# fatchord/WaveRNN

Hardware: AMD Instinct MI355X
Metric: audio samples/sec (real-time factor @22.05 kHz), MoL WaveRNN batched generate (higher is better)
Workload: dtype f32

## Files before the change

### include/wavernn_amd.h

```cpp
#ifndef WAVERNN_AMD_H
#define WAVERNN_AMD_H

#include <stddef.h>
#include <stdint.h>

#ifdef __cplusplus
extern "C" {
#endif

#define WRNN_ABI_VERSION 9

enum {
    WRNN_OK = 0,
    WRNN_ERR_ARG = -1,
    WRNN_ERR_NO_DEVICE = -2,
    WRNN_ERR_HIP = -3,
    WRNN_ERR_WORKSPACE = -4,
    WRNN_ERR_KERNEL = -5,
    WRNN_ERR_RESIDENCY = -6
};

enum { WRNN_MODE_RAW = 0, WRNN_MODE_MOL = 1 };

enum {
    WRNN_ALGO_AUTO = 0,
    WRNN_ALGO_STREAM = 1,
    WRNN_ALGO_LOOP = 2,
    WRNN_ALGO_DUO = 6,
    WRNN_ALGO_CHAIN = 7,
    WRNN_ALGO_OCTO = 8,
    WRNN_ALGO_SPARSE = 5
};

typedef struct wrnn_weights {
    int32_t rnn_dims;
    int32_t fc_dims;
    int32_t feat_dims;
    int32_t aux_dims;
    int32_t n_classes;
    int32_t mode;
    const float *I_w, *I_b;
    const float *w_ih1, *w_hh1, *b_ih1, *b_hh1;
    const float *w_ih2, *w_hh2, *b_ih2, *b_hh2;
    const float *fc1_w, *fc1_b;
    const float *fc2_w, *fc2_b;
    const float *fc3_w, *fc3_b;
} wrnn_weights;

typedef struct wrnn_pack wrnn_pack;

typedef struct wrnn_geometry {
    int32_t B;
    int32_t T;
    int32_t stride;
    int32_t L;
    int32_t hop;
    int32_t n_frames;
} wrnn_geometry;

typedef struct wrnn_timer wrnn_timer;

typedef struct wrnn_run_info {
    const char *kernel;
    int32_t units_per_wg;
    int32_t clusters;
    int32_t depth;
    int32_t rounds;
    int32_t slab_steps;
    int32_t launches;
} wrnn_run_info;

typedef struct wrnn_options {
    int32_t struct_bytes;
    int32_t algo;
    int32_t depth;
    int32_t clusters;
    int32_t cond_valu;
    int32_t slab_steps;
    int32_t t_begin, t_end;
    int32_t tuning;
    const float *force_x;
    float *logits;
    unsigned long long *phase_clocks;
    wrnn_timer *timer;
    wrnn_run_info *info;
    void (*progress)(int32_t steps_done, int32_t T, int32_t n_segments, void *user);
    void *progress_user;
    int32_t mel_stage;
    int32_t mel_rows;
    int32_t mel_scale;
    const float *mel_taps;
    const int32_t *seg_moff;
} wrnn_options;

const char *wrnn_last_error(void);
int wrnn_abi_version(void);

int wrnn_device_cus(int device);

int wrnn_pack_create(const wrnn_weights *w, int device, wrnn_pack **out);
void wrnn_pack_destroy(wrnn_pack *p);
size_t wrnn_pack_weight_bytes(const wrnn_pack *p);
int wrnn_pack_sparse_blocks(const wrnn_pack *p);
int wrnn_pack_sparse_fc_blocks(const wrnn_pack *p);

size_t wrnn_workspace_bytes(const wrnn_pack *p, const wrnn_geometry *g, const wrnn_options *opt);

int wrnn_generate(const wrnn_pack *p, const wrnn_geometry *g, const float *mels_up, const float *aux,
                  const float *noise, float *out, void *workspace, size_t workspace_bytes, const wrnn_options *opt,
                  void *stream);

int wrnn_generate_segments(const wrnn_pack *p, int32_t n_segments, int32_t T, const int32_t *seg_pos,
                           const int32_t *seg_lim, int32_t L, int32_t hop, int32_t n_frames,
                           const float *mels_up, const float *aux, const float *noise, float *out,
                           void *workspace, size_t workspace_bytes, const wrnn_options *opt, void *stream);
size_t wrnn_workspace_bytes_segments(const wrnn_pack *p, int32_t n_segments, int32_t T, int32_t n_frames,
                                     const wrnn_options *opt);

int wrnn_plan_segments(const wrnn_pack *p, int32_t n_segments, int32_t T, const wrnn_options *opt, wrnn_run_info *out);

int wrnn_status(void *workspace, void *stream);

int wrnn_debug_read_exchange(const wrnn_pack *p, void *workspace, int32_t n_segments, int32_t T, int32_t n_frames,
                             const wrnn_options *opt, int cluster, int slot, int layer, int ring, float *host_out);

int wrnn_timer_create(int device, wrnn_timer **out);
void wrnn_timer_destroy(wrnn_timer *t);
float wrnn_timer_ms(wrnn_timer *t);
int wrnn_timer_launches(const wrnn_timer *t);

typedef struct wrnn_pre_weights {
    int32_t feat_dims;
    int32_t compute_dims;
    int32_t res_out_dims;
    int32_t res_blocks;
    int32_t pad;
    int32_t upsample_factors[3];
    const float *conv_in_w;
    const float *bn_in;
    const float *res_w;
    const float *res_bn;
    const float *conv_out_w;
    const float *conv_out_b;
    const float *up_w;
} wrnn_pre_weights;
typedef struct wrnn_pre wrnn_pre;

int wrnn_pre_create(const wrnn_pre_weights *w, int device, wrnn_pre **out);
void wrnn_pre_destroy(wrnn_pre *p);
int wrnn_pre_hop(const wrnn_pre *p);
size_t wrnn_pre_workspace_bytes(const wrnn_pre *p, int32_t n_frames);
int wrnn_pre_upsample(const wrnn_pre *p, const float *mel, int32_t n_frames, float *mels_up, float *aux,
                      void *workspace, size_t workspace_bytes, void *stream);
int wrnn_pre_upsample_rows(const wrnn_pre *p, const float *mel, int32_t n_frames, float *mel_rows, float *aux,
                           void *workspace, size_t workspace_bytes, void *stream);
const char *wrnn_pre_last_error(void);

int wrnn_post_unfold(const float *segments, int32_t T, int32_t n_utt, const int32_t *first, const int32_t *folds,
                     const int64_t *out_off, const double *lut, int32_t n_classes, const double *fade_in,
                     const double *fade_out, int32_t overlap, const double *tail, int32_t tail_len, int32_t batched,
                     double *out, void *stream);
const char *wrnn_post_last_error(void);

typedef struct wrnn_taco_weights {
    uint32_t struct_bytes;
    int32_t n_mels, prenet1, prenet2, decoder_dims, encoder_width, lstm_dims, attn_filters, attn_kernel;
    const float *prenet_fc1_w, *prenet_fc1_b, *prenet_fc2_w, *prenet_fc2_b;
    const float *attn_rnn_w_ih, *attn_rnn_w_hh, *attn_rnn_b_ih, *attn_rnn_b_hh;
    const float *attn_W_w, *attn_W_b, *attn_conv_w, *attn_L_w, *attn_L_b, *attn_v_w;
    const float *rnn_input_w, *rnn_input_b;
    const float *rnn1_w_ih, *rnn1_w_hh, *rnn1_b_ih, *rnn1_b_hh;
    const float *rnn2_w_ih, *rnn2_w_hh, *rnn2_b_ih, *rnn2_b_hh;
    const float *mel_proj_w;
} wrnn_taco_weights;

typedef struct wrnn_taco_call {
    uint32_t struct_bytes;
    int32_t n;
    int32_t r, max_r;
    int32_t max_steps;
    float stop_threshold;
    const float *seq;
    const float *seq_proj;
    float *mel_out;
    float *scores_out;
    int32_t *steps_done;
    void *workspace;
    size_t workspace_bytes;
    void *stream;
    int32_t variant;
} wrnn_taco_call;

size_t wrnn_taco_workspace_bytes(void);
int wrnn_taco_decode(int device, const wrnn_taco_weights *w, const wrnn_taco_call *c);
int wrnn_taco_status(const void *workspace, unsigned *out4, void *stream);
const char *wrnn_taco_last_error(void);

typedef struct wrnn_bigru_call {
    uint32_t struct_bytes;
    int32_t T, hidden;
    const float *gi_fwd, *gi_rev;
    const float *w_hh_fwd, *w_hh_rev;
    const float *b_hh_fwd, *b_hh_rev;
    float *out;
    void *stream;
} wrnn_bigru_call;
int wrnn_bigru(int device, const wrnn_bigru_call *c);

int wrnn_selftest(int device, int which);
float wrnn_selftest_metric(void);

#ifdef __cplusplus
}
#endif
#endif
```

### wavernn_amd/_lib.py

```python
import ctypes
import os
import subprocess

_HERE = os.path.dirname(os.path.abspath(__file__))
CSRC = os.path.join(_HERE, 'csrc')
SO_PATH = os.path.join(CSRC, 'libwavernn_amd.so')

WRNN_OK = 0
ERR_RESIDENCY = -6
MODE_RAW, MODE_MOL = 0, 1
ABI_VERSION = 9
ALGO_AUTO, ALGO_STREAM, ALGO_LOOP, ALGO_SPARSE, ALGO_DUO, ALGO_CHAIN, ALGO_OCTO = 0, 1, 2, 5, 6, 7, 8
ALGOS = {'auto': ALGO_AUTO, 'stream': ALGO_STREAM, 'loop': ALGO_LOOP, 'sparse': ALGO_SPARSE, 'duo': ALGO_DUO, 'chain': ALGO_CHAIN, 'octo': ALGO_OCTO}

EXPORTS = ['wrnn_last_error', 'wrnn_abi_version', 'wrnn_device_cus', 'wrnn_pack_create', 'wrnn_pack_destroy',
           'wrnn_pack_weight_bytes', 'wrnn_pack_sparse_blocks', 'wrnn_pack_sparse_fc_blocks', 'wrnn_workspace_bytes', 'wrnn_workspace_bytes_segments', 'wrnn_generate',
           'wrnn_generate_segments', 'wrnn_plan_segments', 'wrnn_status', 'wrnn_timer_create', 'wrnn_timer_destroy', 'wrnn_timer_ms',
           'wrnn_timer_launches', 'wrnn_debug_read_exchange', 'wrnn_selftest', 'wrnn_selftest_metric', 'wrnn_pre_create',
           'wrnn_pre_destroy', 'wrnn_pre_hop', 'wrnn_pre_workspace_bytes', 'wrnn_pre_upsample', 'wrnn_pre_upsample_rows', 'wrnn_pre_last_error',
           'wrnn_post_unfold', 'wrnn_post_last_error', 'wrnn_taco_workspace_bytes', 'wrnn_taco_decode', 'wrnn_taco_status',
           'wrnn_taco_last_error', 'wrnn_bigru']


class Weights(ctypes.Structure):
    _fields_ = [(n, ctypes.c_int32) for n in ('rnn_dims', 'fc_dims', 'feat_dims', 'aux_dims', 'n_classes', 'mode')] + \
               [(n, ctypes.c_void_p) for n in ('I_w', 'I_b', 'w_ih1', 'w_hh1', 'b_ih1', 'b_hh1', 'w_ih2', 'w_hh2',
                                               'b_ih2', 'b_hh2', 'fc1_w', 'fc1_b', 'fc2_w', 'fc2_b', 'fc3_w', 'fc3_b')]


class PreWeights(ctypes.Structure):
    _fields_ = [(n, ctypes.c_int32) for n in ('feat_dims', 'compute_dims', 'res_out_dims', 'res_blocks', 'pad')] + \
               [('upsample_factors', ctypes.c_int32 * 3)] + \
               [(n, ctypes.c_void_p) for n in ('conv_in_w', 'bn_in', 'res_w', 'res_bn', 'conv_out_w', 'conv_out_b', 'up_w')]


TACO_WEIGHT_FIELDS = ('prenet_fc1_w', 'prenet_fc1_b', 'prenet_fc2_w', 'prenet_fc2_b', 'attn_rnn_w_ih', 'attn_rnn_w_hh', 'attn_rnn_b_ih',
                      'attn_rnn_b_hh', 'attn_W_w', 'attn_W_b', 'attn_conv_w', 'attn_L_w', 'attn_L_b', 'attn_v_w', 'rnn_input_w', 'rnn_input_b',
                      'rnn1_w_ih', 'rnn1_w_hh', 'rnn1_b_ih', 'rnn1_b_hh', 'rnn2_w_ih', 'rnn2_w_hh', 'rnn2_b_ih', 'rnn2_b_hh', 'mel_proj_w')


class TacoWeights(ctypes.Structure):
    _fields_ = [('struct_bytes', ctypes.c_uint32)] + \
               [(n, ctypes.c_int32) for n in ('n_mels', 'prenet1', 'prenet2', 'decoder_dims', 'encoder_width', 'lstm_dims', 'attn_filters',
                                              'attn_kernel')] + \
               [(n, ctypes.c_void_p) for n in TACO_WEIGHT_FIELDS]


class TacoCall(ctypes.Structure):
    _fields_ = [('struct_bytes', ctypes.c_uint32), ('n', ctypes.c_int32), ('r', ctypes.c_int32), ('max_r', ctypes.c_int32),
                ('max_steps', ctypes.c_int32), ('stop_threshold', ctypes.c_float), ('seq', ctypes.c_void_p), ('seq_proj', ctypes.c_void_p),
                ('mel_out', ctypes.c_void_p), ('scores_out', ctypes.c_void_p), ('steps_done', ctypes.c_void_p),
                ('workspace', ctypes.c_void_p), ('workspace_bytes', ctypes.c_size_t), ('stream', ctypes.c_void_p), ('variant', ctypes.c_int32)]


class BigruCall(ctypes.Structure):
    _fields_ = [('struct_bytes', ctypes.c_uint32), ('T', ctypes.c_int32), ('hidden', ctypes.c_int32)] + \
               [(n, ctypes.c_void_p) for n in ('gi_fwd', 'gi_rev', 'w_hh_fwd', 'w_hh_rev', 'b_hh_fwd', 'b_hh_rev', 'out', 'stream')]


class Geometry(ctypes.Structure):
    _fields_ = [(n, ctypes.c_int32) for n in ('B', 'T', 'stride', 'L', 'hop', 'n_frames')]


class RunInfo(ctypes.Structure):
    _fields_ = [('kernel', ctypes.c_char_p)] + \
               [(n, ctypes.c_int32) for n in ('units_per_wg', 'clusters', 'depth', 'rounds', 'slab_steps', 'launches')]


class Options(ctypes.Structure):
    _fields_ = [(n, ctypes.c_int32) for n in ('struct_bytes', 'algo', 'depth', 'clusters', 'cond_valu', 'slab_steps', 't_begin',
                                              't_end', 'tuning')] + \
               [('force_x', ctypes.c_void_p), ('logits', ctypes.c_void_p), ('phase_clocks', ctypes.c_void_p), ('timer', ctypes.c_void_p),
                ('info', ctypes.POINTER(RunInfo)), ('progress', ctypes.c_void_p), ('progress_user', ctypes.c_void_p),
                ('mel_stage', ctypes.c_int32), ('mel_rows', ctypes.c_int32), ('mel_scale', ctypes.c_int32),
                ('mel_taps', ctypes.c_void_p), ('seg_moff', ctypes.c_void_p)]

    def __init__(self, **kw):
        super().__init__(**kw)
        self.struct_bytes = ctypes.sizeof(Options)


PROGRESS_FN = ctypes.CFUNCTYPE(None, ctypes.c_int32, ctypes.c_int32, ctypes.c_int32, ctypes.c_void_p)


class WrnnError(RuntimeError):
    pass


class ResidencyError(WrnnError):
    """WRNN_ERR_RESIDENCY on the FIRST slice of a step-sliced `auto` run: the persistent grid is not co-resident right now.  The
    callers that slice (WaveRNN.generate, generate_corpus) catch it and redo the call unsliced on the stream kernel."""


def build(verbose=False):
    cmd = [os.path.join(CSRC, 'build.sh')]
    res = subprocess.run(cmd, stdout=subprocess.PIPE, stderr=subprocess.STDOUT, text=True)
    if verbose or res.returncode != 0:
        print(res.stdout)
    if res.returncode != 0:
        raise WrnnError('building libwavernn_amd.so failed')
    global _lib
    _lib = None
    return SO_PATH


_lib = None


def lib():
    global _lib
    if _lib is not None:
        return _lib
    if not os.path.exists(SO_PATH):
        raise WrnnError(f'{SO_PATH} not found: run `python -c "import __graft_entry__ as g; g.build()"` '
                        f'(or wavernn_amd/csrc/build.sh).  There is no CPU fallback.')
    import torch
    L = ctypes.CDLL(SO_PATH)
    L.wrnn_last_error.restype = ctypes.c_char_p
    L.wrnn_abi_version.restype = ctypes.c_int
    L.wrnn_device_cus.argtypes = [ctypes.c_int]
    L.wrnn_pack_create.argtypes = [ctypes.POINTER(Weights), ctypes.c_int, ctypes.POINTER(ctypes.c_void_p)]
    L.wrnn_pack_destroy.argtypes = [ctypes.c_void_p]
    L.wrnn_pack_destroy.restype = None
    L.wrnn_pack_weight_bytes.argtypes = [ctypes.c_void_p]
    L.wrnn_pack_weight_bytes.restype = ctypes.c_size_t
    L.wrnn_pack_sparse_blocks.argtypes = [ctypes.c_void_p]
    L.wrnn_pack_sparse_fc_blocks.argtypes = [ctypes.c_void_p]
    L.wrnn_workspace_bytes.argtypes = [ctypes.c_void_p, ctypes.POINTER(Geometry), ctypes.POINTER(Options)]
    L.wrnn_workspace_bytes.restype = ctypes.c_size_t
    L.wrnn_generate.argtypes = [ctypes.c_void_p, ctypes.POINTER(Geometry), ctypes.c_void_p, ctypes.c_void_p,
                                ctypes.c_void_p, ctypes.c_void_p, ctypes.c_void_p, ctypes.c_size_t, ctypes.POINTER(Options),
                                ctypes.c_void_p]
    L.wrnn_workspace_bytes_segments.argtypes = [ctypes.c_void_p, ctypes.c_int32, ctypes.c_int32, ctypes.c_int32,
                                                ctypes.POINTER(Options)]
    L.wrnn_workspace_bytes_segments.restype = ctypes.c_size_t
    L.wrnn_generate_segments.argtypes = [ctypes.c_void_p, ctypes.c_int32, ctypes.c_int32, ctypes.c_void_p, ctypes.c_void_p,
                                         ctypes.c_int32, ctypes.c_int32, ctypes.c_int32, ctypes.c_void_p, ctypes.c_void_p,
                                         ctypes.c_void_p, ctypes.c_void_p, ctypes.c_void_p, ctypes.c_size_t,
                                         ctypes.POINTER(Options), ctypes.c_void_p]
    L.wrnn_plan_segments.argtypes = [ctypes.c_void_p, ctypes.c_int32, ctypes.c_int32, ctypes.POINTER(Options), ctypes.POINTER(RunInfo)]
    L.wrnn_timer_create.argtypes = [ctypes.c_int, ctypes.POINTER(ctypes.c_void_p)]
    L.wrnn_timer_destroy.argtypes = [ctypes.c_void_p]
    L.wrnn_timer_destroy.restype = None
    L.wrnn_timer_ms.argtypes = [ctypes.c_void_p]
    L.wrnn_timer_ms.restype = ctypes.c_float
    L.wrnn_timer_launches.argtypes = [ctypes.c_void_p]
    L.wrnn_debug_read_exchange.argtypes = [ctypes.c_void_p, ctypes.c_void_p, ctypes.c_int32, ctypes.c_int32, ctypes.c_int32,
                                           ctypes.POINTER(Options), ctypes.c_int, ctypes.c_int, ctypes.c_int, ctypes.c_int,
                                           ctypes.c_void_p]
    L.wrnn_pre_create.argtypes = [ctypes.POINTER(PreWeights), ctypes.c_int, ctypes.POINTER(ctypes.c_void_p)]
    L.wrnn_pre_destroy.argtypes = [ctypes.c_void_p]
    L.wrnn_pre_destroy.restype = None
    L.wrnn_pre_hop.argtypes = [ctypes.c_void_p]
    L.wrnn_pre_workspace_bytes.argtypes = [ctypes.c_void_p, ctypes.c_int32]
    L.wrnn_pre_workspace_bytes.restype = ctypes.c_size_t
    L.wrnn_pre_upsample.argtypes = [ctypes.c_void_p, ctypes.c_void_p, ctypes.c_int32, ctypes.c_void_p, ctypes.c_void_p,
                                    ctypes.c_void_p, ctypes.c_size_t, ctypes.c_void_p]
    L.wrnn_pre_upsample_rows.argtypes = L.wrnn_pre_upsample.argtypes
    L.wrnn_pre_last_error.restype = ctypes.c_char_p
    L.wrnn_post_unfold.argtypes = [ctypes.c_void_p, ctypes.c_int32, ctypes.c_int32, ctypes.c_void_p, ctypes.c_void_p, ctypes.c_void_p,
                                   ctypes.c_void_p, ctypes.c_int32, ctypes.c_void_p, ctypes.c_void_p, ctypes.c_int32,
                                   ctypes.c_void_p, ctypes.c_int32, ctypes.c_int32, ctypes.c_void_p, ctypes.c_void_p]
    L.wrnn_post_last_error.restype = ctypes.c_char_p
    L.wrnn_taco_workspace_bytes.restype = ctypes.c_size_t
    L.wrnn_taco_decode.argtypes = [ctypes.c_int, ctypes.POINTER(TacoWeights), ctypes.POINTER(TacoCall)]
    L.wrnn_taco_status.argtypes = [ctypes.c_void_p, ctypes.POINTER(ctypes.c_uint32 * 4), ctypes.c_void_p]
    L.wrnn_taco_last_error.restype = ctypes.c_char_p
    L.wrnn_bigru.argtypes = [ctypes.c_int, ctypes.POINTER(BigruCall)]
    L.wrnn_status.argtypes = [ctypes.c_void_p, ctypes.c_void_p]
    L.wrnn_selftest.argtypes = [ctypes.c_int, ctypes.c_int]
    L.wrnn_selftest_metric.restype = ctypes.c_float
    _lib = L
    return L


def check(rc, what):
    if rc != WRNN_OK:
        raise WrnnError(f'{what} failed (rc={rc}): {lib().wrnn_last_error().decode()}')
```

### wavernn_amd/csrc/wrnn_abi.hip

```cpp
#include <hip/hip_runtime.h>
#include <stdarg.h>
#include <stdio.h>
#include <stdlib.h>
#include <string.h>
#include <math.h>
#include <string>
#include <vector>

#include "../../include/wavernn_amd.h"
#include "wrnn_device.h"

namespace wrnn {
hipError_t launch_cond(const CondArgs &a, int n_cus, bool valu, hipStream_t stream);
hipError_t launch_cond_frames(const CondArgs &a, hipStream_t stream);
hipError_t launch_cond_frames_slab(const CondArgs &a, hipStream_t stream);
hipError_t launch_cond_frag(const CondArgs &a, int n_cus, hipStream_t stream);
hipError_t launch_noise_mol(const float *in, float *out, long n, int B, int n_cus, hipStream_t stream);
hipError_t launch_stream(const LoopArgs &args, int mode, hipStream_t stream);
hipError_t launch_loop(const LoopArgs &args, int ncl, int mode, hipStream_t stream);
int loop_max_depth(int mode);
int loop_clusters(int n_cus);
size_t loop_state_floats(int G);
hipError_t launch_generic(const GenArgs &args, int mode, hipStream_t stream);
bool generic_dims_ok(int H, int F, int M, int A, int C, int mode);
hipError_t launch_duo(const LoopArgs &args, int ncl, int mode, hipStream_t stream);
int duo_clusters(int n_cus);
int duo_max_depth();
size_t duo_xbuf_bytes(int G);
size_t duo_xbuf_bytes_max();
hipError_t launch_sparse(const LoopArgs &args, int nbp, int mode, hipStream_t stream);
int sparse_clusters(int n_cus);
size_t sparse_state_floats();
size_t sparse_xbuf_bytes();
hipError_t launch_put_floats(float *dst, const float *src, int n, hipStream_t stream);
hipError_t launch_chain(const LoopArgs &args, int mode, hipStream_t stream);
hipError_t launch_octo(const LoopArgs &args, int ncl, int mode, hipStream_t stream);
int octo_clusters(int n_cus);
int octo_max_depth();
int chain_clusters(int n_cus);
int chain_max_depth();
size_t chain_state_floats(int G);
size_t chain_xbuf_bytes(int G);
int selftest_mfma(char *msg, size_t n);
int selftest_allgather(int n_cus, char *msg, size_t n, float *us_per_round);
int selftest_tanh(char *msg, size_t n);
int selftest_xor(char *msg, size_t n);
}

using namespace wrnn;

static thread_local char g_err[512] = "";
static void set_err(const char *fmt, ...)
{
    va_list ap;
    va_start(ap, fmt);
    vsnprintf(g_err, sizeof g_err, fmt, ap);
    va_end(ap);
}
#define HIPCHK(expr)                                                                          \
    do {                                                                                      \
        hipError_t e_ = (expr);                                                               \
        if (e_ != hipSuccess) {                                                               \
            set_err("%s failed: %s (%s:%d)", #expr, hipGetErrorString(e_), __FILE__, __LINE__); \
            return WRNN_ERR_HIP;                                                              \
        }                                                                                     \
    } while (0)

struct wrnn_pack {
    int device, n_cus, C, mode;
    size_t weight_bytes;
    char *dev;
    size_t dev_bytes;
    const float *I_w0, *I_b, *I_cT;
    const float *w_ih1, *w_hh1, *b_ih1, *b_hh1, *w_ih2, *w_hh2, *b_ih2, *b_hh2;
    const float *fc1_w, *fc1_b, *fc2_w, *fc2_b, *fc3_w, *fc3_b;
    const float *w_ih1T, *w_hh1T, *w_ih2T, *w_hh2T, *fc1T, *fc2T, *fc3T, *c2_wT, *c3_wT, *c4_wT;
    const float *fc3f;
    const float *u1;
    bool generic;
    int gH, gF, gM, gA;
    const float *g_I_T, *g_fc1T, *g_fc2T, *g_w_ih2T;
    int sp_nbp;
    int sp_max_blocks;
    const float *sp_vals;
    const int *sp_cols;
    int sp_fc_max_blocks;
    const float *sp_fc_vals;
    const int *sp_fc_cols;
};

extern "C" const char *wrnn_last_error(void) { return g_err; }
extern "C" int wrnn_abi_version(void) { return WRNN_ABI_VERSION; }

extern "C" int wrnn_device_cus(int device)
{
    int n = 0;
    if (hipGetDeviceCount(&n) != hipSuccess || n <= 0 || device >= n) {
        set_err("no HIP device %d (count %d)", device, n);
        return WRNN_ERR_NO_DEVICE;
    }
    hipDeviceProp_t prop;
    if (hipGetDeviceProperties(&prop, device) != hipSuccess) return WRNN_ERR_NO_DEVICE;
    return prop.multiProcessorCount;
}

namespace {
struct Builder {
    std::vector<float> host;
    size_t add(const float *src, size_t n)
    {
        size_t off = (host.size() + 63) / 64 * 64;
        host.resize(off + n);
        if (src) memcpy(host.data() + off, src, n * sizeof(float));
        return off;
    }
    size_t add_T(const float *src, int rows, int ld, int col0, int ncols)
    {
        size_t off = add(nullptr, (size_t)ncols * rows);
        float *d = host.data() + off;
        for (int r = 0; r < rows; ++r)
            for (int k = 0; k < ncols; ++k) d[(size_t)k * rows + r] = src[(size_t)r * ld + col0 + k];
        return off;
    }
};
}

extern "C" int wrnn_pack_create(const wrnn_weights *w, int device, wrnn_pack **out)
{
    if (!w || !out) { set_err("NULL argument"); return WRNN_ERR_ARG; }
    const bool shipped = w->rnn_dims == H && w->fc_dims == H && w->feat_dims == MEL && w->aux_dims == AUX;
    const int C = w->n_classes;
    if (w->mode == WRNN_MODE_MOL) {
        if (C != 30) { set_err("MOL needs n_classes == 30"); return WRNN_ERR_ARG; }
    } else if (w->mode == WRNN_MODE_RAW) {
        if (shipped && (C < 2 || C > H)) { set_err("RAW needs 2 <= n_classes <= 512 with the shipped dims"); return WRNN_ERR_ARG; }
    } else { set_err("unknown mode %d", w->mode); return WRNN_ERR_ARG; }
    if (!shipped && !generic_dims_ok(w->rnn_dims, w->fc_dims, w->feat_dims, w->aux_dims, C, w->mode)) {
        set_err("unsupported dims rnn=%d fc=%d feat=%d aux=%d classes=%d: the generic kernel takes rnn, fc, classes <= 2048, feat + aux <= 1024 "
                "(MOL: 30 classes)", w->rnn_dims, w->fc_dims, w->feat_dims, w->aux_dims, C);
        return WRNN_ERR_ARG;
    }
    const float *const *ptrs = &w->I_w;
    for (int i = 0; i < 16; ++i)
        if (!ptrs[i]) { set_err("NULL weight pointer #%d", i); return WRNN_ERR_ARG; }
    const int cus = wrnn_device_cus(device);
    if (cus < 0) return cus;
    DeviceGuard dg(device);
    HIPCHK(dg.err);

    if (!shipped) {
        const int gH = w->rnn_dims, gF = w->fc_dims, gM = w->feat_dims, gA = w->aux_dims;
        Builder b;
        const size_t oI = b.add_T(w->I_w, gH, 1 + gM + gA, 0, 1 + gM + gA), oIb = b.add(w->I_b, gH);
        const size_t o1i = b.add_T(w->w_ih1, 3 * gH, gH, 0, gH), o1h = b.add_T(w->w_hh1, 3 * gH, gH, 0, gH);
        const size_t o1bi = b.add(w->b_ih1, 3 * gH), o1bh = b.add(w->b_hh1, 3 * gH);
        const size_t o2i = b.add_T(w->w_ih2, 3 * gH, gH + gA, 0, gH + gA), o2h = b.add_T(w->w_hh2, 3 * gH, gH, 0, gH);
        const size_t o2bi = b.add(w->b_ih2, 3 * gH), o2bh = b.add(w->b_hh2, 3 * gH);
        const size_t of1 = b.add_T(w->fc1_w, gF, gH + gA, 0, gH + gA), of1b = b.add(w->fc1_b, gF);
        const size_t of2 = b.add_T(w->fc2_w, gF, gF + gA, 0, gF + gA), of2b = b.add(w->fc2_b, gF);
        const size_t of3 = b.add_T(w->fc3_w, C, gF, 0, gF), of3b = b.add(w->fc3_b, C);
        b.add(nullptr, 64);
        wrnn_pack *p = new wrnn_pack();
        memset(p, 0, sizeof *p);
        p->device = device; p->n_cus = cus; p->C = C; p->mode = w->mode; p->generic = true;
        p->gH = gH; p->gF = gF; p->gM = gM; p->gA = gA;
        p->dev_bytes = b.host.size() * sizeof(float);
        p->weight_bytes = sizeof(float) * ((size_t)gH * (1 + gM + gA) + gH + 2 * ((size_t)3 * gH * gH) + (size_t)3 * gH * (gH + gA) + (size_t)3 * gH * gH +
                                           4 * 3 * gH + (size_t)gF * (gH + gA) + (size_t)gF * (gF + gA) + 2 * gF + (size_t)C * gF + C);
        hipError_t e = hipMalloc((void **)&p->dev, p->dev_bytes);
        if (e != hipSuccess) { set_err("hipMalloc(%zu) failed: %s", p->dev_bytes, hipGetErrorString(e)); delete p; return WRNN_ERR_HIP; }
        e = hipMemcpy(p->dev, b.host.data(), p->dev_bytes, hipMemcpyHostToDevice);
        if (e != hipSuccess) { set_err("hipMemcpy failed: %s", hipGetErrorString(e)); (void)hipFree(p->dev); delete p; return WRNN_ERR_HIP; }
        const float *base = (const float *)p->dev;
        p->g_I_T = base + oI; p->I_b = base + oIb;
        p->w_ih1T = base + o1i; p->w_hh1T = base + o1h; p->b_ih1 = base + o1bi; p->b_hh1 = base + o1bh;
        p->g_w_ih2T = base + o2i; p->w_hh2T = base + o2h; p->b_ih2 = base + o2bi; p->b_hh2 = base + o2bh;
        p->g_fc1T = base + of1; p->fc1_b = base + of1b; p->g_fc2T = base + of2; p->fc2_b = base + of2b;
        p->fc3T = base + of3; p->fc3_b = base + of3b;
        p->sp_max_blocks = gH;
        *out = p;
        return WRNN_OK;
    }

    const int KI = 1 + MEL + AUX, K2 = H + AUX;
    Builder b;
    std::vector<float> col0(H);
    for (int r = 0; r < H; ++r) col0[r] = w->I_w[(size_t)r * KI];
    const size_t o_I_w0 = b.add(col0.data(), H), o_I_b = b.add(w->I_b, H);
    const size_t o_I_cT = b.add_T(w->I_w, H, KI, 1, KCOND);
    const size_t o_w_ih1 = b.add(w->w_ih1, (size_t)3 * H * H), o_w_hh1 = b.add(w->w_hh1, (size_t)3 * H * H);
    const size_t o_b_ih1 = b.add(w->b_ih1, 3 * H), o_b_hh1 = b.add(w->b_hh1, 3 * H);
    const size_t o_w_ih2 = b.add(w->w_ih2, (size_t)3 * H * K2), o_w_hh2 = b.add(w->w_hh2, (size_t)3 * H * H);
    const size_t o_b_ih2 = b.add(w->b_ih2, 3 * H), o_b_hh2 = b.add(w->b_hh2, 3 * H);
    const size_t o_fc1_w = b.add(w->fc1_w, (size_t)H * K2), o_fc1_b = b.add(w->fc1_b, H);
    const size_t o_fc2_w = b.add(w->fc2_w, (size_t)H * K2), o_fc2_b = b.add(w->fc2_b, H);
    const size_t o_fc3_w = b.add(w->fc3_w, (size_t)C * H), o_fc3_b = b.add(w->fc3_b, C);
    const size_t o_w_ih1T = b.add_T(w->w_ih1, 3 * H, H, 0, H), o_w_hh1T = b.add_T(w->w_hh1, 3 * H, H, 0, H);
    const size_t o_w_ih2T = b.add_T(w->w_ih2, 3 * H, K2, 0, H), o_w_hh2T = b.add_T(w->w_hh2, 3 * H, H, 0, H);
    const size_t o_fc1T = b.add_T(w->fc1_w, H, K2, 0, H), o_fc2T = b.add_T(w->fc2_w, H, K2, 0, H);
    const size_t o_fc3T = b.add_T(w->fc3_w, C, H, 0, H);
    const size_t o_c2_wT = b.add_T(w->w_ih2, 3 * H, K2, H, AUX);
    const size_t o_c3_wT = b.add_T(w->fc1_w, H, K2, H, AUX), o_c4_wT = b.add_T(w->fc2_w, H, K2, H, AUX);
    size_t o_fc3f = 0;
    if (w->mode == WRNN_MODE_MOL) {
        o_fc3f = b.add(nullptr, (size_t)2 * SEG * H);
        for (int q = 0; q < 2 * SEG * H / 4; ++q) {
            const int l6 = q & 63, r = (q >> 6) & 7, wv = (q >> 9) & 3, tile = q >> 11;
            const int row = 16 * tile + (l6 & 15), kq = l6 >> 4;
            for (int e = 0; e < 4; ++e)
                b.host[o_fc3f + (size_t)q * 4 + e] = row < C ? w->fc3_w[(size_t)row * H + 128 * wv + 16 * r + 4 * kq + e] : 0.f;
        }
    }
    size_t o_u1 = 0;
    {
        o_u1 = b.add(nullptr, (size_t)3 * H);
        for (int r = 0; r < 3 * H; ++r) {
            double acc = 0.0;
            for (int k = 0; k < H; ++k) acc += (double)w->w_ih1[(size_t)r * H + k] * (double)col0[k];
            b.host[o_u1 + r] = (float)acc;
        }
    }
    int sp_nbp = 0, sp_max = 0, sp_fc_max = 0;
    bool sp_fc_ok = false;
    size_t o_spv = 0, o_spc = 0, o_sfv = 0, o_sfc = 0;
    {
        const float *mats[4] = {w->w_ih1, w->w_hh1, w->w_ih2, w->w_hh2};
        const int lds_[4] = {H, H, K2, H};
        std::vector<std::vector<int>> cols((size_t)4 * 32 * 3);
        for (int m = 0; m < 4; ++m)
            for (int wg = 0; wg < 32; ++wg)
                for (int g = 0; g < 3; ++g) {
                    std::vector<int> &cv = cols[((size_t)m * 32 + wg) * 3 + g];
                    const float *base = mats[m] + ((size_t)g * H + 16 * wg) * lds_[m];
                    for (int c = 0; c < H; ++c) {
                        bool nz = false;
                        for (int r = 0; r < 16 && !nz; ++r) nz = base[(size_t)r * lds_[m] + c] != 0.0f;
                        if (nz) cv.push_back(c);
                    }
                    if ((int)cv.size() > sp_max) sp_max = (int)cv.size();
                }
        const float *fmats[2] = {w->fc1_w, w->fc2_w};
        std::vector<std::vector<int>> fcols((size_t)2 * 32);
        for (int m = 0; m < 2; ++m)
            for (int wg = 0; wg < 32; ++wg) {
                std::vector<int> &cv = fcols[(size_t)m * 32 + wg];
                const float *base = fmats[m] + (size_t)(16 * wg) * K2;
                for (int c = 0; c < H; ++c) {
                    bool nz = false;
                    for (int r = 0; r < 16 && !nz; ++r) nz = base[(size_t)r * K2 + c] != 0.0f;
                    if (nz) cv.push_back(c);
                }
                if ((int)cv.size() > sp_fc_max) sp_fc_max = (int)cv.size();
            }
        if (sp_max <= 64 && (w->mode == WRNN_MODE_MOL || C == H)) {
            sp_nbp = sp_max <= 48 ? 48 : 64;
            if (sp_fc_max <= 64) {
                if (sp_fc_max > 48) sp_nbp = 64;
                o_sfv = b.add(nullptr, (size_t)2 * 32 * sp_nbp * 16);
                o_sfc = b.add(nullptr, (size_t)2 * 32 * sp_nbp);
                for (size_t q = 0; q < (size_t)2 * 32 * sp_nbp * 16; ++q) b.host[o_sfv + q] = 0.f;
                int *fi_ = reinterpret_cast<int *>(b.host.data() + o_sfc);
                for (size_t q = 0; q < (size_t)2 * 32 * sp_nbp; ++q) fi_[q] = 0;
                for (int m = 0; m < 2; ++m)
                    for (int wg = 0; wg < 32; ++wg) {
                        const size_t br = (size_t)m * 32 + wg;
                        const std::vector<int> &cv = fcols[br];
                        const float *base = fmats[m] + (size_t)(16 * wg) * K2;
                        for (size_t k = 0; k < cv.size(); ++k) {
                            reinterpret_cast<int *>(b.host.data() + o_sfc)[br * sp_nbp + k] = cv[k];
                            for (int r = 0; r < 16; ++r) b.host[o_sfv + (br * sp_nbp + k) * 16 + r] = base[(size_t)r * K2 + cv[k]];
                        }
                    }
                sp_fc_ok = true;
            }
            o_spv = b.add(nullptr, (size_t)4 * 32 * 3 * sp_nbp * 16);
            o_spc = b.add(nullptr, (size_t)4 * 32 * 3 * sp_nbp);
            for (size_t q = 0; q < (size_t)4 * 32 * 3 * sp_nbp * 16; ++q) b.host[o_spv + q] = 0.f;
            int *ci = reinterpret_cast<int *>(b.host.data() + o_spc);
            for (size_t q = 0; q < (size_t)4 * 32 * 3 * sp_nbp; ++q) ci[q] = 0;
            for (int m = 0; m < 4; ++m)
                for (int wg = 0; wg < 32; ++wg)
                    for (int g = 0; g < 3; ++g) {
                        const size_t br = ((size_t)m * 32 + wg) * 3 + g;
                        const std::vector<int> &cv = cols[br];
                        const float *base = mats[m] + ((size_t)g * H + 16 * wg) * lds_[m];
                        for (size_t k = 0; k < cv.size(); ++k) {
                            ci[br * sp_nbp + k] = cv[k];
                            for (int r = 0; r < 16; ++r) b.host[o_spv + (br * sp_nbp + k) * 16 + r] = base[(size_t)r * lds_[m] + cv[k]];
                        }
                    }
        }
    }
    b.add(nullptr, 64);

    wrnn_pack *p = new wrnn_pack();
    p->device = device; p->n_cus = cus; p->C = C; p->mode = w->mode;
    p->dev_bytes = b.host.size() * sizeof(float);
    p->weight_bytes = sizeof(float) * ((size_t)H * KI + H + 2 * ((size_t)3 * H * H) + (size_t)3 * H * K2 + (size_t)3 * H * H +
                                       4 * 3 * H + 2 * ((size_t)H * K2 + H) + (size_t)C * H + C);
    hipError_t e = hipMalloc((void **)&p->dev, p->dev_bytes);
    if (e != hipSuccess) { set_err("hipMalloc(%zu) failed: %s", p->dev_bytes, hipGetErrorString(e)); delete p; return WRNN_ERR_HIP; }
    e = hipMemcpy(p->dev, b.host.data(), p->dev_bytes, hipMemcpyHostToDevice);
    if (e != hipSuccess) { set_err("hipMemcpy failed: %s", hipGetErrorString(e)); (void)hipFree(p->dev); delete p; return WRNN_ERR_HIP; }
    const float *base = (const float *)p->dev;
    p->I_w0 = base + o_I_w0; p->I_b = base + o_I_b; p->I_cT = base + o_I_cT;
    p->w_ih1 = base + o_w_ih1; p->w_hh1 = base + o_w_hh1; p->b_ih1 = base + o_b_ih1; p->b_hh1 = base + o_b_hh1;
    p->w_ih2 = base + o_w_ih2; p->w_hh2 = base + o_w_hh2; p->b_ih2 = base + o_b_ih2; p->b_hh2 = base + o_b_hh2;
    p->fc1_w = base + o_fc1_w; p->fc1_b = base + o_fc1_b; p->fc2_w = base + o_fc2_w; p->fc2_b = base + o_fc2_b;
    p->fc3_w = base + o_fc3_w; p->fc3_b = base + o_fc3_b;
    p->w_ih1T = base + o_w_ih1T; p->w_hh1T = base + o_w_hh1T; p->w_ih2T = base + o_w_ih2T; p->w_hh2T = base + o_w_hh2T;
    p->fc1T = base + o_fc1T; p->fc2T = base + o_fc2T; p->fc3T = base + o_fc3T;
    p->c2_wT = base + o_c2_wT; p->c3_wT = base + o_c3_wT; p->c4_wT = base + o_c4_wT;
    p->fc3f = w->mode == WRNN_MODE_MOL ? base + o_fc3f : nullptr;
    p->u1 = base + o_u1;
    p->sp_nbp = sp_nbp; p->sp_max_blocks = sp_max;
    p->sp_vals = sp_nbp ? base + o_spv : nullptr;
    p->sp_cols = sp_nbp ? reinterpret_cast<const int *>(base + o_spc) : nullptr;
    p->sp_fc_max_blocks = sp_fc_max;
    p->sp_fc_vals = sp_fc_ok ? base + o_sfv : nullptr;
    p->sp_fc_cols = sp_fc_ok ? reinterpret_cast<const int *>(base + o_sfc) : nullptr;
    *out = p;
    return WRNN_OK;
}

extern "C" void wrnn_pack_destroy(wrnn_pack *p)
{
    if (!p) return;
    (void)hipFree(p->dev);
    delete p;
}

extern "C" size_t wrnn_pack_weight_bytes(const wrnn_pack *p) { return p ? p->weight_bytes : 0; }

extern "C" int wrnn_pack_sparse_blocks(const wrnn_pack *p) { return p ? (p->sp_nbp ? p->sp_max_blocks : -p->sp_max_blocks) : 0; }
extern "C" int wrnn_pack_sparse_fc_blocks(const wrnn_pack *p) { return p ? (p->sp_fc_vals ? p->sp_fc_max_blocks : -p->sp_fc_max_blocks) : 0; }

struct wrnn_timer {
    int device;
    std::vector<hipEvent_t> ev;
    int used;
};

extern "C" int wrnn_timer_create(int device, wrnn_timer **out)
{
    if (!out) { set_err("NULL argument"); return WRNN_ERR_ARG; }
    const int cus = wrnn_device_cus(device);
    if (cus < 0) return cus;
    wrnn_timer *t = new wrnn_timer();
    t->device = device;
    t->used = 0;
    *out = t;
    return WRNN_OK;
}

extern "C" void wrnn_timer_destroy(wrnn_timer *t)
{
    if (!t) return;
    for (hipEvent_t e : t->ev) (void)hipEventDestroy(e);
    delete t;
}

extern "C" int wrnn_timer_launches(const wrnn_timer *t) { return t ? t->used / 2 : 0; }

extern "C" float wrnn_timer_ms(wrnn_timer *t)
{
    if (!t || t->used < 2) return -1.f;
    float total = 0.f;
    for (int i = 0; i + 1 < t->used; i += 2) {
        if (hipEventSynchronize(t->ev[i + 1]) != hipSuccess) return -1.f;
        float ms = 0.f;
        if (hipEventElapsedTime(&ms, t->ev[i], t->ev[i + 1]) != hipSuccess) return -1.f;
        total += ms;
    }
    return total;
}

namespace {
int timer_mark(wrnn_timer *t, hipStream_t stream)
{
    if (!t) return WRNN_OK;
    if (t->used == (int)t->ev.size()) {
        hipEvent_t e;
        HIPCHK(hipEventCreate(&e));
        t->ev.push_back(e);
    }
    HIPCHK(hipEventRecord(t->ev[t->used], stream));
    t->used += 1;
    return WRNN_OK;
}

struct ProgressCtx {
    void (*fn)(int32_t, int32_t, int32_t, void *);
    void *user;
    int32_t done, T, n;
};
void progress_trampoline(void *p)
{
    ProgressCtx *c = static_cast<ProgressCtx *>(p);
    c->fn(c->done, c->T, c->n, c->user);
    delete c;
}
int enqueue_progress(const wrnn_options *o, int done, int T, int n, hipStream_t stream)
{
    if (!o->progress) return WRNN_OK;
    ProgressCtx *c = new ProgressCtx{o->progress, o->progress_user, done, T, n};
    hipError_t e = hipLaunchHostFunc(stream, progress_trampoline, c);
    if (e != hipSuccess) {
        delete c;
        set_err("hipLaunchHostFunc failed: %s", hipGetErrorString(e));
        return WRNN_ERR_HIP;
    }
    return WRNN_OK;
}

enum Kind { K_STREAM, K_LOOP, K_SPARSE, K_DUO, K_GENERIC, K_CHAIN };
constexpr int DUO_TAB_FPS = 8;
constexpr bool DUO_AUTO = true;
constexpr int CHAIN_AUTO_GROUPS = 8;
constexpr bool OCTO_AUTO = false;
constexpr int DUO_MIN_DEPTH = 1;

struct Plan {
    Kind kind;
    int ncl, G, rounds, per_round, slab, ngr_max;
    int tab_fps;
    int t0, t1;
    bool octo;
};

struct WsLayout {
    size_t status, xcc, segs, melc, c2f, c3f, c4f;
    size_t cI, npre;
    size_t xbuf, state, cIf;
    size_t total;
};
size_t al(size_t x) { return (x + 255) / 256 * 256; }

const wrnn_options *norm_options(const wrnn_options *opt, wrnn_options *tmp)
{
    memset(tmp, 0, sizeof *tmp);
    if (opt) {
        size_t n = opt->struct_bytes > 0 ? (size_t)opt->struct_bytes : sizeof *tmp;
        if (n > sizeof *tmp) n = sizeof *tmp;
        memcpy(tmp, opt, n);
    }
    tmp->struct_bytes = (int32_t)sizeof *tmp;
    return tmp;
}

int make_plan(const wrnn_pack *p, int B, int T, const wrnn_options *o, Plan *pl)
{
    const bool shape_ok = (p->mode == WRNN_MODE_MOL) || (p->C == H);
    pl->t0 = o->t_begin; pl->t1 = o->t_end;
    if (pl->t0 == 0 && pl->t1 == 0) pl->t1 = T;
    if (pl->t0 < 0 || pl->t1 > T || pl->t0 >= pl->t1) { set_err("bad step range [%d, %d) of T=%d", pl->t0, pl->t1, T); return WRNN_ERR_ARG; }
    const int algo = o->algo;
    pl->octo = false;
    if (algo != WRNN_ALGO_AUTO && algo != WRNN_ALGO_STREAM && algo != WRNN_ALGO_LOOP && algo != WRNN_ALGO_SPARSE && algo != WRNN_ALGO_DUO && algo != WRNN_ALGO_CHAIN &&
        algo != WRNN_ALGO_OCTO) {
        set_err("unknown algo %d", algo);
        return WRNN_ERR_ARG;
    }
    const int groups = (B + SEG - 1) / SEG;
    pl->kind = K_STREAM; pl->ncl = 0; pl->G = 0; pl->rounds = 1; pl->per_round = B; pl->slab = T; pl->ngr_max = groups;
    if (p->generic) {
        if (algo != WRNN_ALGO_AUTO && algo != WRNN_ALGO_STREAM) {
            set_err("this pack has non-shipped dims (rnn %d, fc %d, feat %d, aux %d): only the generic kernel (algo auto / stream) runs it", p->gH, p->gF, p->gM, p->gA);
            return WRNN_ERR_ARG;
        }
        if (pl->t0 != 0 || pl->t1 != T) { set_err("a partial step range needs a persistent loop kernel"); return WRNN_ERR_ARG; }
        pl->kind = K_GENERIC;
        return WRNN_OK;
    }
    const int ccl = chain_clusters(p->n_cus);
    const bool chain_hw = shape_ok && ccl >= 1;
    if (algo == WRNN_ALGO_CHAIN && !chain_hw) {
        set_err("wrnn_chain_kernel needs MOL or RAW with 512 classes, and >= 256 CUs (C = %d, device: %d CUs)", p->C, p->n_cus);
        return !shape_ok ? WRNN_ERR_ARG : WRNN_ERR_RESIDENCY;
    }
    const bool sparse_auto = p->sp_nbp && p->mode == WRNN_MODE_MOL;
    if (algo == WRNN_ALGO_CHAIN || (algo == WRNN_ALGO_AUTO && chain_hw && groups <= CHAIN_AUTO_GROUPS && !sparse_auto)) {
        const int gmax = chain_max_depth();
        int g = o->depth;
        if (g < 1 || g > gmax) {
            const int rounds = (groups + ccl * gmax - 1) / (ccl * gmax);
            g = (groups + ccl * rounds - 1) / (ccl * rounds);
            if (g < 1) g = 1;
            if (g > gmax) g = gmax;
        }
        pl->kind = K_CHAIN; pl->ncl = ccl; pl->G = g;
        pl->rounds = (groups + ccl * g - 1) / (ccl * g);
        pl->per_round = (B + pl->rounds - 1) / pl->rounds;
        pl->ngr_max = (pl->per_round + SEG - 1) / SEG;
        if (pl->ngr_max > ccl * g) { pl->rounds += 1; pl->per_round = (B + pl->rounds - 1) / pl->rounds; pl->ngr_max = (pl->per_round + SEG - 1) / SEG; }
        int slab = o->slab_steps;
        if (slab < 1) {
            slab = p->mode == WRNN_MODE_MOL ? (int)((32u << 20) / ((size_t)pl->per_round * 11 * sizeof(float) * pl->rounds)) : 4096;
            if (slab < 16) slab = 16;
            if (slab > 4096) slab = 4096;
        }
        if (slab > T) slab = T;
        pl->slab = slab;
        pl->tab_fps = DUO_TAB_FPS;
    }
    const int scl = sparse_clusters(p->n_cus);
    if (algo == WRNN_ALGO_SPARSE && (!p->sp_nbp || scl < 1)) {
        set_err("block-sparse kernel needs MOL or RAW with 512 classes, >= 256 CUs and GRU matrices with <= 64 surviving 16x1 blocks per block row "
                "(this pack: mode %s, %d classes, up to %d blocks; device: %d CUs)", p->mode == WRNN_MODE_MOL ? "MOL" : "RAW", p->C, p->sp_max_blocks, p->n_cus);
        return (!p->sp_nbp) ? WRNN_ERR_ARG : WRNN_ERR_RESIDENCY;
    }
    if (pl->kind == K_CHAIN) {
    } else if (algo == WRNN_ALGO_SPARSE || (algo == WRNN_ALGO_AUTO && sparse_auto && scl >= 1)) {
        pl->kind = K_SPARSE; pl->ncl = scl; pl->G = 1;
        pl->rounds = (groups + scl - 1) / scl;
        pl->per_round = (B + pl->rounds - 1) / pl->rounds;
        pl->ngr_max = (pl->per_round + SEG - 1) / SEG;
        if (pl->ngr_max > scl) { pl->rounds += 1; pl->per_round = (B + pl->rounds - 1) / pl->rounds; pl->ngr_max = (pl->per_round + SEG - 1) / SEG; }
        int slab = o->slab_steps;
        if (slab < 1) {
            slab = p->mode == WRNN_MODE_MOL ? (int)((32u << 20) / ((size_t)pl->per_round * 11 * sizeof(float) * pl->rounds)) : 4096;
            if (slab < 16) slab = 16;
            if (slab > 4096) slab = 4096;
        }
        if (slab > T) slab = T;
        pl->slab = slab;
        pl->tab_fps = DUO_TAB_FPS;
    } else if (algo == WRNN_ALGO_AUTO || algo == WRNN_ALGO_LOOP || algo == WRNN_ALGO_DUO || algo == WRNN_ALGO_OCTO) {
        int ncl = loop_clusters(p->n_cus);
        if (algo == WRNN_ALGO_OCTO && (p->mode != WRNN_MODE_MOL || octo_clusters(p->n_cus) != MAXCL)) {
            set_err("wrnn_octo_kernel needs MOL and >= 256 CUs (mode %d, device has %d CUs)", p->mode, p->n_cus);
            return p->mode != WRNN_MODE_MOL ? WRNN_ERR_ARG : WRNN_ERR_RESIDENCY;
        }
        if (algo == WRNN_ALGO_DUO && (!shape_ok || duo_clusters(p->n_cus) < 1)) {
            set_err("the two-workgroups-per-CU loop kernel needs MOL or RAW with 512 classes, and >= 64 CUs (C = %d, device has %d CUs)", p->C, p->n_cus);
            return !shape_ok ? WRNN_ERR_ARG : WRNN_ERR_RESIDENCY;
        }
        if (shape_ok && ncl >= 1) {
            if (o->clusters == 1 || o->clusters == 2 || o->clusters == 4) ncl = o->clusters < ncl ? o->clusters : ncl;
            else if (groups < ncl && !(DUO_AUTO && algo != WRNN_ALGO_LOOP && ncl == MAXCL)) {
                int c2 = 1; while (c2 < groups) c2 *= 2; if (c2 < ncl) ncl = c2;
            }
            const int gmax = algo == WRNN_ALGO_OCTO ? octo_max_depth() : loop_max_depth(p->mode);
            int g = o->depth;
            if (g < 1 || g > gmax) {
                const int rounds = (groups + ncl * gmax - 1) / (ncl * gmax);
                g = (groups + ncl * rounds - 1) / (ncl * rounds);
                if (g < 1) g = 1;
                if (g > gmax) g = gmax;
            }
            pl->kind = K_LOOP; pl->ncl = ncl; pl->G = g;
            if (algo == WRNN_ALGO_DUO || algo == WRNN_ALGO_OCTO || (algo == WRNN_ALGO_AUTO && DUO_AUTO && g >= DUO_MIN_DEPTH && ncl == MAXCL))
                pl->kind = K_DUO;
            pl->octo = pl->kind == K_DUO && (algo == WRNN_ALGO_OCTO || (algo == WRNN_ALGO_AUTO && OCTO_AUTO && p->mode == WRNN_MODE_MOL && ncl == MAXCL && !o->clusters));
            pl->rounds = (groups + ncl * g - 1) / (ncl * g);
            pl->per_round = (B + pl->rounds - 1) / pl->rounds;
            pl->ngr_max = (pl->per_round + SEG - 1) / SEG;
            if (pl->ngr_max > ncl * g) { pl->rounds += 1; pl->per_round = (B + pl->rounds - 1) / pl->rounds; pl->ngr_max = (pl->per_round + SEG - 1) / SEG; }
            int slab = o->slab_steps;
            if (slab < 1) {
                if (pl->kind == K_DUO) slab = p->mode == WRNN_MODE_MOL ? (int)((32u << 20) / ((size_t)pl->per_round * 11 * sizeof(float) * pl->rounds)) : 4096;
                else slab = (int)((96u << 20) / ((size_t)pl->ngr_max * SEG * H * sizeof(float)));
                if (slab < 16) slab = 16;
                if (slab > (pl->kind == K_DUO ? 4096 : 1024)) slab = pl->kind == K_DUO ? 4096 : 1024;
            }
            if (slab > T) slab = T;
            pl->slab = slab;
            pl->tab_fps = DUO_TAB_FPS;
        } else if (algo == WRNN_ALGO_LOOP) {
            set_err("the loop kernel needs >= 64 CUs and (MOL or RAW with 512 classes); device has %d CUs, C=%d", p->n_cus, p->C);
            return WRNN_ERR_RESIDENCY;
        }
    }
    if (pl->kind != K_LOOP && pl->kind != K_DUO && pl->kind != K_SPARSE && pl->kind != K_CHAIN && (pl->t0 != 0 || pl->t1 != T)) {
        set_err("a partial step range [%d, %d) needs a persistent loop kernel", pl->t0, pl->t1);
        return WRNN_ERR_ARG;
    }
    if ((pl->kind == K_DUO || pl->kind == K_SPARSE || pl->kind == K_CHAIN) && ((size_t)B * pl->tab_fps + 1) * 3 * H * sizeof(float) >= 0x7FFFF000ull) {
        set_err("%d segments in one call: the per-slab aux tables exceed a 2 GB buffer resource; split the call (generate_corpus caps a launch at 4096 segments)", B);
        return WRNN_ERR_ARG;
    }
    return WRNN_OK;
}

WsLayout ws_layout(const wrnn_pack *p, const Plan &pl, int B, int T, int n_frames)
{
    WsLayout l;
    memset(&l, 0, sizeof l);
    size_t o = 0;
    l.status = o; o = al(o + STATUS_WORDS * sizeof(unsigned));
    l.xcc = o;    o = al(o + XCC_WORDS * sizeof(unsigned));
    l.segs = o;   o = al(o + (size_t)3 * B * sizeof(int));
    l.melc = o;   o = al(o + (size_t)3 * LAST_SCALE * sizeof(float));
    if (pl.kind == K_GENERIC) { l.total = o; return l; }
    const bool slabbed = pl.kind == K_DUO || pl.kind == K_SPARSE || pl.kind == K_CHAIN;
    const size_t tab_rows = slabbed ? (size_t)B * pl.tab_fps + 1 : (size_t)n_frames + 1;
    l.c2f = o;    o = al(o + tab_rows * 3 * H * sizeof(float));
    l.c3f = o;    o = al(o + tab_rows * H * sizeof(float));
    l.c4f = o;    o = al(o + tab_rows * H * sizeof(float));
    const bool mol = p->mode == WRNN_MODE_MOL;
    if (pl.kind == K_LOOP || slabbed) {
        l.xbuf = o;  o = al(o + (pl.kind == K_CHAIN ? chain_xbuf_bytes(pl.G) : pl.kind == K_SPARSE ? sparse_xbuf_bytes() : slabbed ? duo_xbuf_bytes_max() : XBUF_FLOATS * sizeof(float)));
        l.state = o; o = al(o + (size_t)pl.rounds * (pl.kind == K_SPARSE ? sparse_state_floats() : pl.kind == K_CHAIN ? chain_state_floats(pl.G) : loop_state_floats(pl.G)) * sizeof(float));
        l.cIf = o;   if (pl.kind == K_LOOP) o = al(o + (size_t)pl.slab * pl.ngr_max * SEG * H * sizeof(float));
        l.npre = o;  if (mol) o = al(o + (size_t)pl.slab * 11 * B * sizeof(float));
    } else {
        l.cI = o;    o = al(o + (size_t)T * B * H * sizeof(float));
        l.npre = o;
    }
    l.total = o;
    return l;
}
void hop_magic(int hop, unsigned *magic, int *shift)
{
    *magic = 0u; *shift = 0;
    if (hop < 2) return;
    int s = 0;
    while ((1ll << s) < hop) ++s;
    const unsigned long long m = ((1ull << (31 + s)) + (unsigned long long)hop - 1ull) / (unsigned long long)hop;
    if (m >> 32) return;
    const int sh = s - 1;
    for (long long q = 0; q * hop < (1ll << 31); q += 997) {
        for (long long p = q * hop - 1; p <= q * hop + 1; ++p) {
            if (p < 0 || p >= (1ll << 31)) continue;
            if ((long long)(((unsigned long long)p * m) >> (32 + sh)) != p / hop) return;
        }
    }
    *magic = (unsigned)m; *shift = sh;
}

int check_geometry(const wrnn_geometry *g)
{
    if (!g) { set_err("NULL geometry"); return WRNN_ERR_ARG; }
    if (g->B < 1 || g->T < 1 || g->L < 1 || g->hop < 1 || g->n_frames < 1 || g->stride < 0) {
        set_err("bad geometry B=%d T=%d stride=%d L=%d hop=%d n_frames=%d", g->B, g->T, g->stride, g->L, g->hop, g->n_frames);
        return WRNN_ERR_ARG;
    }
    if ((long)g->n_frames * g->hop < g->L) { set_err("n_frames*hop < L"); return WRNN_ERR_ARG; }
    if ((double)g->B * g->stride + g->T > 2.0e9) { set_err("geometry overflows int32"); return WRNN_ERR_ARG; }
    return WRNN_OK;
}
int check_segments(int B, int T, const int32_t *seg_pos, const int32_t *seg_lim, int L, int hop, int n_frames)
{
    if (B < 1 || T < 1 || L < 1 || hop < 1 || n_frames < 1 || !seg_pos || !seg_lim) {
        set_err("bad segment table B=%d T=%d L=%d hop=%d n_frames=%d", B, T, L, hop, n_frames);
        return WRNN_ERR_ARG;
    }
    if ((long)n_frames * hop < L) { set_err("n_frames*hop < L"); return WRNN_ERR_ARG; }
    for (int b = 0; b < B; ++b) {
        if (seg_pos[b] < 0 || seg_lim[b] < 0 || seg_lim[b] > L || (double)seg_pos[b] + T > 2.0e9) {
            set_err("segment %d: pos=%d lim=%d outside [0,%d]", b, seg_pos[b], seg_lim[b], L);
            return WRNN_ERR_ARG;
        }
    }
    return WRNN_OK;
}
}

extern "C" size_t wrnn_workspace_bytes_segments(const wrnn_pack *p, int32_t n_segments, int32_t T, int32_t n_frames,
                                                const wrnn_options *opt)
{
    if (!p || n_segments < 1 || T < 1 || n_frames < 1) return 0;
    wrnn_options tmp;
    const wrnn_options *o = norm_options(opt, &tmp);
    Plan pl;
    wrnn_options whole = *o;
    whole.t_begin = 0; whole.t_end = 0;
    if (make_plan(p, n_segments, T, &whole, &pl) != WRNN_OK) return 0;
    return ws_layout(p, pl, n_segments, T, n_frames).total;
}

extern "C" int wrnn_plan_segments(const wrnn_pack *p, int32_t n_segments, int32_t T, const wrnn_options *opt, wrnn_run_info *out)
{
    if (!p || !out || n_segments < 1 || T < 1) { set_err("bad argument"); return WRNN_ERR_ARG; }
    wrnn_options tmp;
    wrnn_options whole = *norm_options(opt, &tmp);
    whole.t_begin = 0; whole.t_end = 0;
    Plan pl;
    int rc = make_plan(p, n_segments, T, &whole, &pl);
    if (rc != WRNN_OK) return rc;
    memset(out, 0, sizeof *out);
    out->kernel = pl.kind == K_GENERIC ? "wrnn_generic_kernel" : pl.kind == K_CHAIN ? "wrnn_chain_kernel" : pl.kind == K_DUO ? (pl.octo ? "wrnn_octo_kernel" : "wrnn_duo_kernel") : pl.kind == K_LOOP ? "wrnn_loop_kernel" : (pl.kind == K_SPARSE ? "wrnn_sparse_kernel" : "wrnn_stream_kernel");
    out->units_per_wg = pl.kind == K_STREAM ? 0 : (pl.kind == K_SPARSE ? 64 : 16);
    out->clusters = pl.ncl; out->depth = pl.G; out->rounds = pl.rounds; out->slab_steps = pl.slab;
    return WRNN_OK;
}

extern "C" size_t wrnn_workspace_bytes(const wrnn_pack *p, const wrnn_geometry *g, const wrnn_options *opt)
{
    if (!p || check_geometry(g) != WRNN_OK) return 0;
    return wrnn_workspace_bytes_segments(p, g->B, g->T, g->n_frames, opt);
}

extern "C" int wrnn_generate_segments(const wrnn_pack *p, int32_t B, int32_t T, const int32_t *seg_pos,
                                      const int32_t *seg_lim, int32_t L, int32_t hop, int32_t n_frames,
                                      const float *mels_up, const float *aux, const float *noise, float *out,
                                      void *workspace, size_t workspace_bytes, const wrnn_options *opt, void *stream_)
{
    if (!p || !mels_up || !aux || !noise || !out || !workspace) { set_err("NULL argument"); return WRNN_ERR_ARG; }
    int rc = check_segments(B, T, seg_pos, seg_lim, L, hop, n_frames);
    if (rc != WRNN_OK) return rc;
    wrnn_options tmp;
    const wrnn_options *o = norm_options(opt, &tmp);
    Plan pl;
    {
        wrnn_options whole = *o;
        whole.t_begin = 0; whole.t_end = 0;
        if ((rc = make_plan(p, B, T, &whole, &pl)) != WRNN_OK) return rc;
        pl.t0 = o->t_begin; pl.t1 = o->t_end;
        if (pl.t0 == 0 && pl.t1 == 0) pl.t1 = T;
        if (pl.t0 < 0 || pl.t1 > T || pl.t0 >= pl.t1) { set_err("bad step range [%d, %d) of T=%d", pl.t0, pl.t1, T); return WRNN_ERR_ARG; }
        if (pl.kind != K_LOOP && pl.kind != K_DUO && pl.kind != K_SPARSE && pl.kind != K_CHAIN && (pl.t0 != 0 || pl.t1 != T)) { set_err("a partial step range needs a persistent loop kernel"); return WRNN_ERR_ARG; }
    }
    const WsLayout l = ws_layout(p, pl, B, T, n_frames);
    if (workspace_bytes < l.total) { set_err("workspace %zu < required %zu", workspace_bytes, l.total); return WRNN_ERR_WORKSPACE; }
    if (((uintptr_t)workspace & 255) != 0) { set_err("workspace must be 256-byte aligned"); return WRNN_ERR_ARG; }
    hipStream_t stream = (hipStream_t)stream_;
    DeviceGuard dg(p->device);
    HIPCHK(dg.err);
    char *ws = (char *)workspace;
    wrnn_timer *timer = o->timer;
    if (timer && pl.t0 == 0) timer->used = 0;

    if (pl.t0 == 0) HIPCHK(hipMemsetAsync(ws + l.status, 0, STATUS_WORDS * sizeof(unsigned), stream));
    HIPCHK(hipMemcpyAsync(ws + l.segs, seg_pos, (size_t)B * sizeof(int), hipMemcpyHostToDevice, stream));
    HIPCHK(hipMemcpyAsync(ws + l.segs + (size_t)B * sizeof(int), seg_lim, (size_t)B * sizeof(int), hipMemcpyHostToDevice, stream));
    const int *d_pos = (const int *)(ws + l.segs), *d_lim = d_pos + B;
    if (o->mel_stage) {
        if (pl.kind != K_DUO && pl.kind != K_SPARSE && pl.kind != K_CHAIN) { set_err("wrnn_options.mel_stage: only wrnn_duo_kernel / wrnn_sparse_kernel / wrnn_chain_kernel form the last up-sampling stage (this call runs on another kernel)"); return WRNN_ERR_ARG; }
        if (o->mel_stage != 1 || o->mel_scale != LAST_SCALE || !o->mel_taps || !o->seg_moff || o->mel_rows < 3) {
            set_err("wrnn_options.mel_stage=%d: needs mel_scale == %d (got %d), mel_taps, seg_moff, mel_rows >= 3", o->mel_stage, LAST_SCALE, o->mel_scale);
            return WRNN_ERR_ARG;
        }
        for (int b = 0; b < B; ++b) {
            const long last = (seg_lim[b] < (long)seg_pos[b] + T ? seg_lim[b] : (long)seg_pos[b] + T) - 1;
            if (last < seg_pos[b]) continue;
            const long j0 = (long)seg_pos[b] + o->seg_moff[b], j1 = last + o->seg_moff[b];
            if (o->seg_moff[b] < 0 || j0 / LAST_SCALE < 1 || j1 / LAST_SCALE + 1 >= o->mel_rows) {
                set_err("segment %d: positions %ld..%ld of the last up-sampling stage reach outside its %d input rows", b, j0, j1, o->mel_rows);
                return WRNN_ERR_ARG;
            }
        }
        float coef[3 * LAST_SCALE];
        for (int ph = 0; ph < LAST_SCALE; ++ph) {
            double c0 = 0, c1 = 0, c2 = 0;
            for (int j = 0; j <= 2 * LAST_SCALE; ++j) {
                const double w = o->mel_taps[j];
                if (j < LAST_SCALE - ph) c0 += w; else if (j < 2 * LAST_SCALE - ph) c1 += w; else c2 += w;
            }
            coef[3 * ph] = (float)c0; coef[3 * ph + 1] = (float)c1; coef[3 * ph + 2] = (float)c2;
        }
        HIPCHK(hipMemcpyAsync(ws + l.segs + (size_t)2 * B * sizeof(int), o->seg_moff, (size_t)B * sizeof(int), hipMemcpyHostToDevice, stream));
        HIPCHK(launch_put_floats((float *)(ws + l.melc), coef, 3 * LAST_SCALE, stream));
    }
    if (pl.kind == K_GENERIC) {
        GenArgs g;
        memset(&g, 0, sizeof g);
        g.I_T = p->g_I_T; g.I_b = p->I_b; g.w_ih1T = p->w_ih1T; g.w_hh1T = p->w_hh1T; g.b_ih1 = p->b_ih1; g.b_hh1 = p->b_hh1;
        g.w_ih2T = p->g_w_ih2T; g.w_hh2T = p->w_hh2T; g.b_ih2 = p->b_ih2; g.b_hh2 = p->b_hh2;
        g.fc1T = p->g_fc1T; g.fc1_b = p->fc1_b; g.fc2T = p->g_fc2T; g.fc2_b = p->fc2_b; g.fc3T = p->fc3T; g.fc3_b = p->fc3_b;
        g.mels_up = mels_up; g.aux = aux; g.noise = noise; g.force_x = o->force_x; g.out = out; g.dbg_logits = o->logits;
        g.seg_pos = d_pos; g.seg_lim = d_lim;
        g.H = p->gH; g.F = p->gF; g.M = p->gM; g.A = p->gA; g.C = p->C; g.B = B; g.T = T; g.hop = hop;
        if ((rc = timer_mark(timer, stream)) != WRNN_OK) return rc;
        HIPCHK(launch_generic(g, p->mode, stream));
        if ((rc = timer_mark(timer, stream)) != WRNN_OK) return rc;
        wrnn_run_info gi;
        memset(&gi, 0, sizeof gi);
        gi.kernel = "wrnn_generic_kernel"; gi.rounds = 1; gi.slab_steps = T; gi.launches = 1;
        if (o->info) *o->info = gi;
        return enqueue_progress(o, T, T, B, stream);
    }

    CondArgs c;
    memset(&c, 0, sizeof c);
    c.mels_up = mels_up; c.aux = aux; c.I_cT = p->I_cT; c.I_b = p->I_b; c.c2_wT = p->c2_wT; c.b_ih2 = p->b_ih2;
    c.c3_wT = p->c3_wT; c.fc1_b = p->fc1_b; c.c4_wT = p->c4_wT; c.fc2_b = p->fc2_b;
    c.c2f = (float *)(ws + l.c2f); c.c3f = (float *)(ws + l.c3f); c.c4f = (float *)(ws + l.c4f);
    c.seg_pos = d_pos; c.seg_lim = d_lim;
    c.B = B; c.T = T; c.hop = hop; c.NF = n_frames;
    const bool slabbed = pl.kind == K_DUO || pl.kind == K_SPARSE || pl.kind == K_CHAIN;
    if (slabbed) {
        const long eff = (long)(pl.tab_fps - 2) * hop + 1;
        if (pl.slab > eff) pl.slab = (int)eff;
    } else HIPCHK(launch_cond_frames(c, stream));

    LoopArgs a;
    memset(&a, 0, sizeof a);
    a.I_w0 = p->I_w0; a.w_ih1 = p->w_ih1; a.w_hh1 = p->w_hh1; a.b_ih1 = p->b_ih1; a.b_hh1 = p->b_hh1;
    a.w_ih2 = p->w_ih2; a.w_hh2 = p->w_hh2; a.b_hh2 = p->b_hh2; a.fc1_w = p->fc1_w; a.fc2_w = p->fc2_w;
    a.fc3_w = p->fc3_w; a.fc3_b = p->fc3_b; a.fc3f = p->fc3f; a.u1 = p->u1;
    a.w_ih1T = p->w_ih1T; a.w_hh1T = p->w_hh1T; a.w_ih2T = p->w_ih2T; a.w_hh2T = p->w_hh2T;
    a.fc1T = p->fc1T; a.fc2T = p->fc2T; a.fc3T = p->fc3T;
    a.c2f = c.c2f; a.c3f = c.c3f; a.c4f = c.c4f;
    a.noise = noise; a.force_x = o->force_x; a.out = out; a.dbg_logits = o->logits;
    a.status = (unsigned *)(ws + l.status);
    a.prof = (u64 *)o->phase_clocks;
    a.tuning = o->tuning;
    a.seg_pos = d_pos; a.seg_lim = d_lim;
    a.Btot = B; a.T = T; a.hop = hop; a.NF = n_frames; a.C = p->C;
    a.NG = (B + SEG - 1) / SEG;
    a.Nall = B;
    a.xcc_tab = (unsigned *)(ws + l.xcc);
    a.mels_up = mels_up; a.aux_fr = aux; a.I_cT = p->I_cT; a.I_b = p->I_b;
    a.mel_stage = o->mel_stage; a.seg_moff = d_pos + 2 * B; a.mel_coef = (const float *)(ws + l.melc);
    hop_magic(hop, &a.hop_magic, &a.hop_shift);

    wrnn_run_info info;
    memset(&info, 0, sizeof info);
    info.clusters = pl.ncl; info.depth = pl.G; info.rounds = pl.rounds; info.slab_steps = pl.slab;

    if (pl.kind == K_LOOP || slabbed) {
        const bool duo = slabbed, sparse = pl.kind == K_SPARSE, chain = pl.kind == K_CHAIN;
        const bool octo = pl.kind == K_DUO && pl.octo;
        info.kernel = chain ? "wrnn_chain_kernel" : sparse ? "wrnn_sparse_kernel" : (duo ? (octo ? "wrnn_octo_kernel" : "wrnn_duo_kernel") : "wrnn_loop_kernel"); info.units_per_wg = sparse ? 64 : 16;
        a.sp_vals = p->sp_vals; a.sp_cols = p->sp_cols;
        a.sp_fc_vals = (o->tuning & 2048) ? nullptr : p->sp_fc_vals; a.sp_fc_cols = p->sp_fc_cols;
        const bool mol = p->mode == WRNN_MODE_MOL;
        a.xbuf = (float *)(ws + l.xbuf);
        a.cIf = (const float *)(ws + l.cIf);
        a.G = pl.G;
        c.cI = (float *)(ws + l.cIf);
        for (int s0 = pl.t0; s0 < pl.t1; s0 += pl.slab) {
            const int s1 = s0 + pl.slab < pl.t1 ? s0 + pl.slab : pl.t1;
            if (mol) {
                HIPCHK(launch_noise_mol(noise + (size_t)(s0 - pl.t0) * 11 * B, (float *)(ws + l.npre), (long)(s1 - s0) * 11 * B, B, p->n_cus, stream));
                a.noise_pre = (const float *)(ws + l.npre);
                a.noise_t0 = s0;
            } else {
                a.noise_t0 = pl.t0;
            }
            if (duo) {
                c.t0 = s0; c.B = B; c.FPS = pl.tab_fps;
                HIPCHK(launch_cond_frames_slab(c, stream));
                a.tab_fps = pl.tab_fps; a.tab_t0 = s0;
            }
            for (int r = 0; r < pl.rounds; ++r) {
                const int rb0 = (int)(((long)r * B) / pl.rounds), rb1 = (int)(((long)(r + 1) * B) / pl.rounds);
                const int nr = rb1 - rb0;
                if (nr < 1) continue;
                const int ngr = (nr + SEG - 1) / SEG;
                c.t0 = s0; c.t1 = s1; c.rb0 = rb0; c.B = nr; c.NG = ngr;
                if (!duo) HIPCHK(launch_cond_frag(c, p->n_cus, stream));
                if (!duo) HIPCHK(hipMemsetAsync(ws + l.xbuf, 0xFF, XBUF_FLOATS * sizeof(float), stream));
                else if (s0 == 0 || pl.rounds > 1 || (o->tuning & 4)) HIPCHK(hipMemsetAsync(ws + l.xbuf, 0xFF, chain ? chain_xbuf_bytes(pl.G) : sparse ? sparse_xbuf_bytes() : duo_xbuf_bytes(pl.G), stream));
                if (duo) HIPCHK(hipMemsetAsync(ws + l.xcc, 0, XCC_WORDS * sizeof(unsigned), stream));
                a.state = (float *)(ws + l.state) + (size_t)r * (sparse ? sparse_state_floats() : chain ? chain_state_floats(pl.G) : loop_state_floats(pl.G));
                a.t0 = s0; a.t1 = s1; a.cI_t0 = s0; a.rb0 = rb0; a.Btot = nr; a.NG = ngr; a.resume = s0 > 0 ? 1 : 0;
                a.kind_tag = chain ? 4 : sparse ? 3 : (duo ? (octo ? 5 : 2) : 1);
                if ((rc = timer_mark(timer, stream)) != WRNN_OK) return rc;
                hipError_t e = chain ? launch_chain(a, p->mode, stream) : sparse ? launch_sparse(a, p->sp_nbp, p->mode, stream) : (duo ? (octo ? launch_octo(a, pl.ncl, p->mode, stream) : launch_duo(a, pl.ncl, p->mode, stream)) : launch_loop(a, pl.ncl, p->mode, stream));
                if (e != hipSuccess) {
                    (void)hipGetLastError();
                    set_err("%s cooperative launch failed: %s", info.kernel, hipGetErrorString(e));
                    return e == hipErrorCooperativeLaunchTooLarge ? WRNN_ERR_RESIDENCY : WRNN_ERR_HIP;
                }
                if ((rc = timer_mark(timer, stream)) != WRNN_OK) return rc;
                info.launches += 1;
            }
            if ((rc = enqueue_progress(o, s1, T, B, stream)) != WRNN_OK) return rc;
        }
    } else {
        c.cI = (float *)(ws + l.cI);
        a.cI = c.cI;
        HIPCHK(launch_cond(c, p->n_cus, o->cond_valu != 0, stream));
        info.kernel = "wrnn_stream_kernel";
        a.b0 = 0;
        a.nb = B;
        if ((rc = timer_mark(timer, stream)) != WRNN_OK) return rc;
        HIPCHK(launch_stream(a, p->mode, stream));
        if ((rc = timer_mark(timer, stream)) != WRNN_OK) return rc;
        info.launches = 1;
        if ((rc = enqueue_progress(o, T, T, B, stream)) != WRNN_OK) return rc;
    }
    if (o->info) *o->info = info;
    return WRNN_OK;
}

extern "C" int wrnn_generate(const wrnn_pack *p, const wrnn_geometry *g, const float *mels_up, const float *aux,
                             const float *noise, float *out, void *workspace, size_t workspace_bytes, const wrnn_options *opt,
                             void *stream_)
{
    int rc = check_geometry(g);
    if (rc != WRNN_OK) return rc;
    std::vector<int32_t> pos(g->B), lim(g->B, g->L);
    for (int b = 0; b < g->B; ++b) pos[b] = b * g->stride;
    return wrnn_generate_segments(p, g->B, g->T, pos.data(), lim.data(), g->L, g->hop, g->n_frames, mels_up, aux,
                                  noise, out, workspace, workspace_bytes, opt, stream_);
}

extern "C" int wrnn_status(void *workspace, void *stream)
{
    if (!workspace) { set_err("NULL workspace"); return WRNN_ERR_ARG; }
    HIPCHK(hipStreamSynchronize((hipStream_t)stream));
    unsigned st[STATUS_WORDS];
    HIPCHK(hipMemcpy(st, workspace, sizeof st, hipMemcpyDeviceToHost));
    if (st[0] != 0 || st[1] != 0) {
        set_err("loop kernel gave up: code 0x%x (phase %u) workgroup %u step %u thread %u", st[1], st[1] & 0xff, st[2], st[3], st[4]);
        return WRNN_ERR_KERNEL;
    }
    return WRNN_OK;
}

extern "C" int wrnn_debug_read_exchange(const wrnn_pack *p, void *workspace, int32_t n_segments, int32_t T, int32_t n_frames,
                                        const wrnn_options *opt, int cluster, int slot, int layer, int ring, float *host_out)
{
    if (!p || !workspace || !host_out) { set_err("NULL argument"); return WRNN_ERR_ARG; }
    wrnn_options tmp;
    wrnn_options whole = *norm_options(opt, &tmp);
    whole.t_begin = 0; whole.t_end = 0;
    Plan pl;
    int rc = make_plan(p, n_segments, T, &whole, &pl);
    if (rc != WRNN_OK) return rc;
    if (pl.kind != K_LOOP || cluster < 0 || cluster >= MAXCL || slot < 0 || slot >= LMAXG || layer < 0 || layer >= NXLAYER || ring < 0 || ring >= XRING) {
        set_err("no such exchange layer");
        return WRNN_ERR_ARG;
    }
    const WsLayout l = ws_layout(p, pl, n_segments, T, n_frames);
    HIPCHK(hipDeviceSynchronize());
    std::vector<float> frag((size_t)SEG * H);
    const size_t off = ((((size_t)cluster * LMAXG + slot) * NXLAYER + layer) * XRING + ring) * SEG * H;
    HIPCHK(hipMemcpy(frag.data(), (char *)workspace + l.xbuf + off * sizeof(float), frag.size() * sizeof(float), hipMemcpyDeviceToHost));
    for (int j = 0; j < SEG; ++j)
        for (int k = 0; k < H; ++k) {
            const int w = k >> 7, r = (k >> 4) & 7, kq = (k >> 2) & 3, e = k & 3;
            host_out[(size_t)j * H + k] = frag[(size_t)(((w * 8 + r) * 64 + kq * 16 + j) * 4 + e)];
        }
    return WRNN_OK;
}

static float g_selftest_metric = -1.f;
extern "C" float wrnn_selftest_metric(void) { return g_selftest_metric; }

extern "C" int wrnn_selftest(int device, int which)
{
    const int cus = wrnn_device_cus(device);
    if (cus < 0) return cus;
    DeviceGuard dg(device);
    HIPCHK(dg.err);
    char msg[400] = "";
    int rc;
    if (which == 1) rc = selftest_mfma(msg, sizeof msg);
    else if (which == 2) rc = selftest_allgather(cus, msg, sizeof msg, &g_selftest_metric);
    else if (which == 3) rc = selftest_tanh(msg, sizeof msg);
    else if (which == 4) rc = selftest_xor(msg, sizeof msg);
    else { set_err("unknown selftest %d", which); return WRNN_ERR_ARG; }
    if (rc != 0) { set_err("selftest %d failed: %s", which, msg); return WRNN_ERR_KERNEL; }
    set_err("selftest %d ok: %s", which, msg);
    return WRNN_OK;
}
```

### wavernn_amd/csrc/wrnn_cond.hip

```cpp
#include <stdlib.h>
#include <string.h>

#include "wrnn_device.h"

namespace wrnn {


constexpr int CR = 8;

__global__ __launch_bounds__(H) void wrnn_cond_sample_kernel(const CondArgs a)
{
    __shared__ __attribute__((aligned(16))) float in[CR][KCOND];
    const int r = threadIdx.x;
    float wreg[KCOND];
#pragma unroll
    for (int k = 0; k < KCOND; ++k) wreg[k] = a.I_cT[k * H + r];
    const float bias = a.I_b[r];
    const long rows = (long)a.T * a.B;
    for (long base = (long)blockIdx.x * CR; base < rows; base += (long)gridDim.x * CR) {
        __syncthreads();
        for (int q = r; q < CR * KCOND; q += H) {
            const int rr = q / KCOND, k = q % KCOND;
            const long row = base + rr;
            float val = 0.f;
            if (row < rows) {
                const int t = (int)(row / a.B), b = (int)(row % a.B);
                const int p = a.seg_pos[b] + t;
                if (p < a.seg_lim[b]) val = (k < MEL) ? a.mels_up[(size_t)p * MEL + k] : a.aux[(size_t)(p / a.hop) * 4 * AUX + (k - MEL)];
            }
            in[rr][k] = val;
        }
        __syncthreads();
#pragma unroll
        for (int rr = 0; rr < CR; ++rr) {
            float acc = 0.f;
#pragma unroll
            for (int k = 0; k < KCOND; k += 4) {
                const float4 x = *reinterpret_cast<const float4 *>(&in[rr][k]);
                acc = fmaf(wreg[k + 0], x.x, acc);
                acc = fmaf(wreg[k + 1], x.y, acc);
                acc = fmaf(wreg[k + 2], x.z, acc);
                acc = fmaf(wreg[k + 3], x.w, acc);
            }
            if (base + rr < rows) a.cI[(size_t)(base + rr) * H + r] = acc + bias;
        }
    }
}


constexpr int CKB = KCOND / 16;
constexpr int CLD = KCOND + 4;
__global__ __launch_bounds__(256, 1) void wrnn_cond_mfma_kernel(const CondArgs a)
{
    __shared__ __attribute__((aligned(16))) float in[16 * CLD];
    const int tid = threadIdx.x, lane = tid & 63, w = tid >> 6;
    const int fi = lane & 15, kq = lane >> 4;
    float A[8][4 * CKB];
    float4 bias[8];
#pragma unroll
    for (int tt = 0; tt < 8; ++tt) {
        const int row = 128 * w + 16 * tt + fi;
#pragma unroll
        for (int r = 0; r < CKB; ++r)
#pragma unroll
            for (int e = 0; e < 4; ++e) A[tt][4 * r + e] = a.I_cT[(size_t)(16 * r + 4 * kq + e) * H + row];
        bias[tt] = *reinterpret_cast<const float4 *>(a.I_b + 128 * w + 16 * tt + 4 * kq);
    }
    const long rows = (long)a.T * a.B;
    for (long base = (long)blockIdx.x * 16; base < rows; base += (long)gridDim.x * 16) {
        __syncthreads();
        for (int q = tid; q < 16 * KCOND; q += 256) {
            const int rr = q / KCOND, k = q % KCOND;
            const long row = base + rr;
            float val = 0.f;
            if (row < rows) {
                const int t = (int)(row / a.B), b = (int)(row % a.B);
                const int p = a.seg_pos[b] + t;
                if (p < a.seg_lim[b]) val = (k < MEL) ? a.mels_up[(size_t)p * MEL + k] : a.aux[(size_t)(p / a.hop) * 4 * AUX + (k - MEL)];
            }
            in[rr * CLD + k] = val;
        }
        __syncthreads();
        float4 bf[CKB];
#pragma unroll
        for (int r = 0; r < CKB; ++r) bf[r] = *reinterpret_cast<const float4 *>(in + fi * CLD + 16 * r + 4 * kq);
        f32x4 acc[8];
#pragma unroll
        for (int tt = 0; tt < 8; ++tt) acc[tt] = f32x4{0.f, 0.f, 0.f, 0.f};
#pragma unroll
        for (int r = 0; r < CKB; ++r) {
#pragma unroll
            for (int tt = 0; tt < 8; ++tt) acc[tt] = __builtin_amdgcn_mfma_f32_16x16x4f32(A[tt][4 * r + 0], bf[r].x, acc[tt], 0, 0, 0);
#pragma unroll
            for (int tt = 0; tt < 8; ++tt) acc[tt] = __builtin_amdgcn_mfma_f32_16x16x4f32(A[tt][4 * r + 1], bf[r].y, acc[tt], 0, 0, 0);
#pragma unroll
            for (int tt = 0; tt < 8; ++tt) acc[tt] = __builtin_amdgcn_mfma_f32_16x16x4f32(A[tt][4 * r + 2], bf[r].z, acc[tt], 0, 0, 0);
#pragma unroll
            for (int tt = 0; tt < 8; ++tt) acc[tt] = __builtin_amdgcn_mfma_f32_16x16x4f32(A[tt][4 * r + 3], bf[r].w, acc[tt], 0, 0, 0);
        }
        if (base + fi < rows) {
#pragma unroll
            for (int tt = 0; tt < 8; ++tt) {
                const float4 o = make_float4(acc[tt][0] + bias[tt].x, acc[tt][1] + bias[tt].y, acc[tt][2] + bias[tt].z, acc[tt][3] + bias[tt].w);
                *reinterpret_cast<float4 *>(a.cI + (size_t)(base + fi) * H + 128 * w + 16 * tt + 4 * kq) = o;
            }
        }
    }
}

__global__ __launch_bounds__(256, 1) void wrnn_cond_frag_kernel(const CondArgs a)
{
    __shared__ __attribute__((aligned(16))) float in[16 * CLD];
    const int tid = threadIdx.x, lane = tid & 63, w = tid >> 6;
    const int fi = lane & 15, kq = lane >> 4;
    float A[8][4 * CKB];
    float4 bias[8];
#pragma unroll
    for (int tt = 0; tt < 8; ++tt) {
        const int row = 128 * w + 16 * tt + fi;
#pragma unroll
        for (int r = 0; r < CKB; ++r)
#pragma unroll
            for (int e = 0; e < 4; ++e) A[tt][4 * r + e] = a.I_cT[(size_t)(16 * r + 4 * kq + e) * H + row];
        bias[tt] = *reinterpret_cast<const float4 *>(a.I_b + 128 * w + 16 * tt + 4 * kq);
    }
    const long tiles = (long)(a.t1 - a.t0) * a.NG;
    constexpr int NQ = (16 * KCOND + 255) / 256;
    auto gather = [&](long tile, float (&v)[NQ]) {
        const int t = a.t0 + (int)(tile / a.NG), g = (int)(tile % a.NG);
        const int b0 = a.rb0 + (int)(((long)g * a.B) / a.NG), nb = a.rb0 + (int)(((long)(g + 1) * a.B) / a.NG) - b0;
#pragma unroll
        for (int i = 0; i < NQ; ++i) {
            const int q = tid + 256 * i;
            const int rr = q / KCOND, k = q % KCOND;
            float val = 0.f;
            if (q < 16 * KCOND && rr < nb) {
                const int p = a.seg_pos[b0 + rr] + t;
                if (p < a.seg_lim[b0 + rr]) val = (k < MEL) ? a.mels_up[(size_t)p * MEL + k] : a.aux[(size_t)(p / a.hop) * 4 * AUX + (k - MEL)];
            }
            v[i] = val;
        }
    };
    float cur[NQ] = {}, nxt[NQ] = {};
    if (blockIdx.x < tiles) gather(blockIdx.x, cur);
    for (long tile = blockIdx.x; tile < tiles; tile += gridDim.x) {
        __syncthreads();
#pragma unroll
        for (int i = 0; i < NQ; ++i) {
            const int q = tid + 256 * i;
            if (q < 16 * KCOND) in[(q / KCOND) * CLD + q % KCOND] = cur[i];
        }
        __syncthreads();
        if (tile + gridDim.x < tiles) gather(tile + gridDim.x, nxt);
        float4 bf[CKB];
#pragma unroll
        for (int r = 0; r < CKB; ++r) bf[r] = *reinterpret_cast<const float4 *>(in + fi * CLD + 16 * r + 4 * kq);
        f32x4 acc[8];
#pragma unroll
        for (int tt = 0; tt < 8; ++tt) acc[tt] = f32x4{0.f, 0.f, 0.f, 0.f};
#pragma unroll
        for (int r = 0; r < CKB; ++r) {
#pragma unroll
            for (int tt = 0; tt < 8; ++tt) acc[tt] = __builtin_amdgcn_mfma_f32_16x16x4f32(A[tt][4 * r + 0], bf[r].x, acc[tt], 0, 0, 0);
#pragma unroll
            for (int tt = 0; tt < 8; ++tt) acc[tt] = __builtin_amdgcn_mfma_f32_16x16x4f32(A[tt][4 * r + 1], bf[r].y, acc[tt], 0, 0, 0);
#pragma unroll
            for (int tt = 0; tt < 8; ++tt) acc[tt] = __builtin_amdgcn_mfma_f32_16x16x4f32(A[tt][4 * r + 2], bf[r].z, acc[tt], 0, 0, 0);
#pragma unroll
            for (int tt = 0; tt < 8; ++tt) acc[tt] = __builtin_amdgcn_mfma_f32_16x16x4f32(A[tt][4 * r + 3], bf[r].w, acc[tt], 0, 0, 0);
        }
        float4 *dst = reinterpret_cast<float4 *>(a.cI + (size_t)tile * (SEG * H)) + (w * 8) * 64 + lane;
#pragma unroll
        for (int tt = 0; tt < 8; ++tt)
            dst[tt * 64] = make_float4(acc[tt][0] + bias[tt].x, acc[tt][1] + bias[tt].y, acc[tt][2] + bias[tt].z, acc[tt][3] + bias[tt].w);
#pragma unroll
        for (int i = 0; i < NQ; ++i) cur[i] = nxt[i];
    }
}

__global__ __launch_bounds__(H) void wrnn_cond_frame_kernel(const CondArgs a)
{
    __shared__ float ax[4 * AUX];
    const int f = blockIdx.x, r = threadIdx.x;
    if (r < 4 * AUX) ax[r] = (f < a.NF) ? a.aux[(size_t)f * 4 * AUX + r] : 0.f;
    __syncthreads();
    float g0 = 0.f, g1 = 0.f, g2 = 0.f, y3 = 0.f, y4 = 0.f;
#pragma unroll 8
    for (int k = 0; k < AUX; ++k) {
        g0 = fmaf(a.c2_wT[k * 3 * H + r], ax[AUX + k], g0);
        g1 = fmaf(a.c2_wT[k * 3 * H + H + r], ax[AUX + k], g1);
        g2 = fmaf(a.c2_wT[k * 3 * H + 2 * H + r], ax[AUX + k], g2);
        y3 = fmaf(a.c3_wT[k * H + r], ax[2 * AUX + k], y3);
        y4 = fmaf(a.c4_wT[k * H + r], ax[3 * AUX + k], y4);
    }
    a.c2f[(size_t)f * 3 * H + r] = g0 + a.b_ih2[r];
    a.c2f[(size_t)f * 3 * H + H + r] = g1 + a.b_ih2[H + r];
    a.c2f[(size_t)f * 3 * H + 2 * H + r] = g2 + a.b_ih2[2 * H + r];
    a.c3f[(size_t)f * H + r] = y3 + a.fc1_b[r];
    a.c4f[(size_t)f * H + r] = y4 + a.fc2_b[r];
}

__global__ __launch_bounds__(H) void wrnn_cond_frame_slab_kernel(const CondArgs a)
{
    __shared__ float ax[4 * AUX];
    const int row = blockIdx.x, r = threadIdx.x;
    int f = a.NF;
    if (row < a.B * a.FPS) {
        const int b = row / a.FPS, j = row % a.FPS;
        f = (a.seg_pos[b] + a.t0) / a.hop + j;
    }
    if (r < 4 * AUX) ax[r] = (f < a.NF) ? a.aux[(size_t)f * 4 * AUX + r] : 0.f;
    __syncthreads();
    float g0 = 0.f, g1 = 0.f, g2 = 0.f, y3 = 0.f, y4 = 0.f;
#pragma unroll 8
    for (int k = 0; k < AUX; ++k) {
        g0 = fmaf(a.c2_wT[k * 3 * H + r], ax[AUX + k], g0);
        g1 = fmaf(a.c2_wT[k * 3 * H + H + r], ax[AUX + k], g1);
        g2 = fmaf(a.c2_wT[k * 3 * H + 2 * H + r], ax[AUX + k], g2);
        y3 = fmaf(a.c3_wT[k * H + r], ax[2 * AUX + k], y3);
        y4 = fmaf(a.c4_wT[k * H + r], ax[3 * AUX + k], y4);
    }
    a.c2f[(size_t)row * 3 * H + r] = g0 + a.b_ih2[r];
    a.c2f[(size_t)row * 3 * H + H + r] = g1 + a.b_ih2[H + r];
    a.c2f[(size_t)row * 3 * H + 2 * H + r] = g2 + a.b_ih2[2 * H + r];
    a.c3f[(size_t)row * H + r] = y3 + a.fc1_b[r];
    a.c4f[(size_t)row * H + r] = y4 + a.fc2_b[r];
}

__global__ __launch_bounds__(256) void wrnn_noise_mol_kernel(const float *__restrict__ in, float *__restrict__ out, long n, int B)
{
    const long stride = (long)gridDim.x * blockDim.x;
    for (long i = (long)blockIdx.x * blockDim.x + threadIdx.x; i < n; i += stride) {
        const float u = in[i];
        const int col = (int)(i % (11L * B));
        out[i] = (col < 10 * B) ? logf(-logf(u)) : (logf(u) - logf(1.0f - u));
    }
}

hipError_t launch_noise_mol(const float *in, float *out, long n, int B, int n_cus, hipStream_t stream)
{
    long blocks = (n + 255) / 256;
    if (blocks > (long)n_cus * 8) blocks = (long)n_cus * 8;
    if (blocks < 1) blocks = 1;
    hipLaunchKernelGGL(wrnn_noise_mol_kernel, dim3((unsigned)blocks), dim3(256), 0, stream, in, out, n, B);
    return hipGetLastError();
}

hipError_t launch_cond_frames(const CondArgs &a, hipStream_t stream)
{
    hipLaunchKernelGGL(wrnn_cond_frame_kernel, dim3(a.NF + 1), dim3(H), 0, stream, a);
    return hipGetLastError();
}

hipError_t launch_cond_frames_slab(const CondArgs &a, hipStream_t stream)
{
    hipLaunchKernelGGL(wrnn_cond_frame_slab_kernel, dim3(a.B * a.FPS + 1), dim3(H), 0, stream, a);
    return hipGetLastError();
}

struct PutFloats { float v[64]; };
__global__ void wrnn_put_floats_kernel(float *dst, PutFloats src, int n)
{
    if ((int)threadIdx.x < n) dst[threadIdx.x] = src.v[threadIdx.x];
}
hipError_t launch_put_floats(float *dst, const float *src, int n, hipStream_t stream)
{
    if (n < 1 || n > 64) return hipErrorInvalidValue;
    PutFloats p;
    for (int i = 0; i < 64; ++i) p.v[i] = i < n ? src[i] : 0.f;
    hipLaunchKernelGGL(wrnn_put_floats_kernel, dim3(1), dim3(64), 0, stream, dst, p, n);
    return hipGetLastError();
}

hipError_t launch_cond_frag(const CondArgs &a, int n_cus, hipStream_t stream)
{
    long blocks = (long)(a.t1 - a.t0) * a.NG;
    if (blocks > n_cus) blocks = n_cus;
    if (blocks < 1) blocks = 1;
    hipLaunchKernelGGL(wrnn_cond_frag_kernel, dim3((unsigned)blocks), dim3(256), 0, stream, a);
    return hipGetLastError();
}

hipError_t launch_cond(const CondArgs &a, int n_cus, bool valu, hipStream_t stream)
{
    const long rows = (long)a.T * a.B;
    if (valu) {
        long blocks = (rows + CR - 1) / CR;
        const long cap = (long)n_cus * 4;
        if (blocks > cap) blocks = cap;
        if (blocks < 1) blocks = 1;
        hipLaunchKernelGGL(wrnn_cond_sample_kernel, dim3((unsigned)blocks), dim3(H), 0, stream, a);
    } else {
        long blocks = (rows + 15) / 16;
        if (blocks > n_cus) blocks = n_cus;
        if (blocks < 1) blocks = 1;
        hipLaunchKernelGGL(wrnn_cond_mfma_kernel, dim3((unsigned)blocks), dim3(256), 0, stream, a);
    }
    return hipGetLastError();
}

}
```

### wavernn_amd/csrc/wrnn_pre.hip

```cpp
#include <math.h>
#include <stdio.h>
#include <string.h>
#include <vector>

#include "wrnn_device.h"
#include "../../include/wavernn_amd.h"

namespace wrnn {

constexpr int PC = 128;
constexpr int PFEAT = MEL;
constexpr int PK = 5;
constexpr int PPAD = 2;
constexpr int PKIN = PFEAT * PK;
constexpr int PLDI = 516;
constexpr int PLDX = 132;
constexpr int PNF = 16;

struct PreArgs {
    const float *mel;
    const float *conv_in_w;
    const float *bn_in;
    const float *res_w;
    const float *res_bn;
    const float *conv_out_w;
    const float *conv_out_b;
    float *aux;
    int N, blocks;
};

__device__ __forceinline__ f32x4 pre_tile(const float *W, int ld, int kvalid, int row0, int nchunks, const float *act, int lda,
                                          int lane)
{
    const int fi = lane & 15, kq = lane >> 4;
    f32x4 total = {0.f, 0.f, 0.f, 0.f};
    for (int kc = 0; kc < nchunks; ++kc) {
        float a[AF];
#pragma unroll
        for (int r = 0; r < AF / 4; ++r) {
            const int col = kc * 128 + 16 * r + 4 * kq;
            float4 v = make_float4(0.f, 0.f, 0.f, 0.f);
            if (col < kvalid) v = *reinterpret_cast<const float4 *>(W + (size_t)(row0 + fi) * ld + col);
            a[4 * r + 0] = v.x; a[4 * r + 1] = v.y; a[4 * r + 2] = v.z; a[4 * r + 3] = v.w;
        }
        const f32x4 part = mfma_tile(a, act + fi * lda + kc * 128 + 4 * kq);
        total = (kc == 0) ? part : total + part;
    }
    return total;
}

__global__ __launch_bounds__(256) void wrnn_resnet_kernel(const PreArgs a)
{
    __shared__ __attribute__((aligned(16))) float XIN[PNF * PLDI];
    __shared__ __attribute__((aligned(16))) float XA[PNF * PLDX];
    __shared__ __attribute__((aligned(16))) float XB[PNF * PLDX];
    const int tid = threadIdx.x, lane = tid & 63, w = tid >> 6;
    const int j0 = blockIdx.x * PNF;
    const int N = a.N;
    for (int q = tid; q < PNF * PLDI; q += 256) {
        const int j = q / PLDI, k = q % PLDI;
        float v = 0.f;
        if (k < PKIN) {
            const int c = k / PK, t = k % PK;
            const int f = j0 + j + t - PPAD;
            if (f >= 0 && f < N && j0 + j < N) v = a.mel[(size_t)c * N + f];
        }
        XIN[q] = v;
    }
    __syncthreads();
    const int fi = lane & 15, rq = (lane >> 4) * 4;
#pragma unroll
    for (int tt = 0; tt < 2; ++tt) {
        const int row0 = 32 * w + 16 * tt;
        const f32x4 d = pre_tile(a.conv_in_w, PKIN, PKIN, row0, 4, XIN, PLDI, lane);
        const float4 s = *reinterpret_cast<const float4 *>(a.bn_in + row0 + rq);
        const float4 t = *reinterpret_cast<const float4 *>(a.bn_in + PC + row0 + rq);
        float4 y;
        y.x = fmaxf(fmaf(d[0], s.x, t.x), 0.f); y.y = fmaxf(fmaf(d[1], s.y, t.y), 0.f);
        y.z = fmaxf(fmaf(d[2], s.z, t.z), 0.f); y.w = fmaxf(fmaf(d[3], s.w, t.w), 0.f);
        *reinterpret_cast<float4 *>(XA + fi * PLDX + row0 + rq) = y;
    }
    __syncthreads();
    for (int b = 0; b < a.blocks; ++b) {
        const float *W1 = a.res_w + (size_t)(2 * b) * PC * PC, *W2 = W1 + PC * PC;
        const float *bn1 = a.res_bn + (size_t)(2 * b) * 2 * PC, *bn2 = bn1 + 2 * PC;
#pragma unroll
        for (int tt = 0; tt < 2; ++tt) {
            const int row0 = 32 * w + 16 * tt;
            const f32x4 d = pre_tile(W1, PC, PC, row0, 1, XA, PLDX, lane);
            const float4 s = *reinterpret_cast<const float4 *>(bn1 + row0 + rq);
            const float4 t = *reinterpret_cast<const float4 *>(bn1 + PC + row0 + rq);
            float4 y;
            y.x = fmaxf(fmaf(d[0], s.x, t.x), 0.f); y.y = fmaxf(fmaf(d[1], s.y, t.y), 0.f);
            y.z = fmaxf(fmaf(d[2], s.z, t.z), 0.f); y.w = fmaxf(fmaf(d[3], s.w, t.w), 0.f);
            *reinterpret_cast<float4 *>(XB + fi * PLDX + row0 + rq) = y;
        }
        __syncthreads();
        f32x4 d2[2];
#pragma unroll
        for (int tt = 0; tt < 2; ++tt) d2[tt] = pre_tile(W2, PC, PC, 32 * w + 16 * tt, 1, XB, PLDX, lane);
#pragma unroll
        for (int tt = 0; tt < 2; ++tt) {
            const int row0 = 32 * w + 16 * tt;
            const float4 s = *reinterpret_cast<const float4 *>(bn2 + row0 + rq);
            const float4 t = *reinterpret_cast<const float4 *>(bn2 + PC + row0 + rq);
            float4 r = *reinterpret_cast<float4 *>(XA + fi * PLDX + row0 + rq);
            r.x += fmaf(d2[tt][0], s.x, t.x); r.y += fmaf(d2[tt][1], s.y, t.y);
            r.z += fmaf(d2[tt][2], s.z, t.z); r.w += fmaf(d2[tt][3], s.w, t.w);
            *reinterpret_cast<float4 *>(XA + fi * PLDX + row0 + rq) = r;
        }
        __syncthreads();
    }
#pragma unroll
    for (int tt = 0; tt < 2; ++tt) {
        const int row0 = 32 * w + 16 * tt;
        const f32x4 d = pre_tile(a.conv_out_w, PC, PC, row0, 1, XA, PLDX, lane);
        const float4 bo = *reinterpret_cast<const float4 *>(a.conv_out_b + row0 + rq);
        if (j0 + fi < N)
            *reinterpret_cast<float4 *>(a.aux + (size_t)(j0 + fi) * PC + row0 + rq) = make_float4(d[0] + bo.x, d[1] + bo.y, d[2] + bo.z, d[3] + bo.w);
    }
}

struct GenPreArgs {
    PreArgs p;
    int feat, C, R, pad, gf;
};
__global__ __launch_bounds__(256) void wrnn_resnet_generic_kernel(const GenPreArgs g)
{
    extern __shared__ __attribute__((aligned(16))) float gsm[];
    const PreArgs &a = g.p;
    const int feat = g.feat, C = g.C, R = g.R, pad = g.pad, GF = g.gf, K = 2 * pad + 1, WW = GF + 2 * pad;
    float *MW = gsm, *XA = MW + feat * WW, *XB = XA + GF * C;
    const int tid = threadIdx.x, N = a.N;
    const int j0 = blockIdx.x * GF;
    for (int q = tid; q < feat * WW; q += 256) {
        const int c = q / WW, f = j0 + q % WW - pad;
        MW[q] = (f >= 0 && f < N) ? a.mel[(size_t)c * N + f] : 0.f;
    }
    __syncthreads();
    for (int o = tid; o < C * GF; o += 256) {
        const int c = o / GF, j = o % GF;
        const float *wr = a.conv_in_w + (size_t)c * feat * K;
        float acc = 0.f;
        for (int ci = 0; ci < feat; ++ci)
            for (int t = 0; t < K; ++t) acc = fmaf(wr[ci * K + t], MW[ci * WW + j + t], acc);
        XA[j * C + c] = fmaxf(fmaf(acc, a.bn_in[c], a.bn_in[C + c]), 0.f);
    }
    __syncthreads();
    for (int b = 0; b < a.blocks; ++b) {
        const float *W1 = a.res_w + (size_t)(2 * b) * C * C, *W2 = W1 + (size_t)C * C;
        const float *bn1 = a.res_bn + (size_t)(2 * b) * 2 * C, *bn2 = bn1 + 2 * C;
        for (int o = tid; o < C * GF; o += 256) {
            const int c = o / GF, j = o % GF;
            float acc = 0.f;
            for (int k = 0; k < C; ++k) acc = fmaf(W1[(size_t)c * C + k], XA[j * C + k], acc);
            XB[j * C + c] = fmaxf(fmaf(acc, bn1[c], bn1[C + c]), 0.f);
        }
        __syncthreads();
        for (int o = tid; o < C * GF; o += 256) {
            const int c = o / GF, j = o % GF;
            float acc = 0.f;
            for (int k = 0; k < C; ++k) acc = fmaf(W2[(size_t)c * C + k], XB[j * C + k], acc);
            XA[j * C + c] += fmaf(acc, bn2[c], bn2[C + c]);
        }
        __syncthreads();
    }
    for (int o = tid; o < R * GF; o += 256) {
        const int r = o / GF, j = o % GF;
        float acc = 0.f;
        for (int k = 0; k < C; ++k) acc = fmaf(a.conv_out_w[(size_t)r * C + k], XA[j * C + k], acc);
        if (j0 + j < N) a.aux[(size_t)(j0 + j) * R + r] = acc + a.conv_out_b[r];
    }
}

template <bool FIRST, bool LAST, int S, int F = PFEAT>
__global__ __launch_bounds__(256) void wrnn_upstage_kernel(const float *__restrict__ in, float *__restrict__ out,
                                                           const float *__restrict__ taps, int n_in, int s_rt, int pad, int indent, int feat_rt = PFEAT)
{
    const int s = S > 0 ? S : s_rt;
    const int feat = F > 0 ? F : feat_rt;
    const long n_out = (long)n_in * s;
    const long total = LAST ? (n_out - 2L * indent) * feat : n_out * feat;
    const int ld_in = FIRST ? n_in - 2 * pad : n_in;
    for (long idx = (long)blockIdx.x * blockDim.x + threadIdx.x; idx < total; idx += (long)gridDim.x * blockDim.x) {
        int c;
        long q;
        if (LAST) { c = (int)(idx % feat); q = idx / feat + indent; }
        else { c = (int)(idx / n_out); q = idx % n_out; }
        float acc = 0.f;
#pragma unroll
        for (int j = 0; j <= 2 * s; ++j) {
            const long u = q + j - s;
            float v = 0.f;
            if (u >= 0 && u < n_out) {
                int f = (int)(u / s);
                if (FIRST) { f -= pad; v = (f >= 0 && f < ld_in) ? in[(size_t)c * ld_in + f] : 0.f; }
                else v = in[(size_t)c * ld_in + f];
            }
            acc = fmaf(taps[j], v, acc);
        }
        if (LAST) out[(size_t)(q - indent) * feat + c] = acc;
        else out[(size_t)c * n_out + q] = acc;
    }
}

template <int S>
__global__ __launch_bounds__(256) void wrnn_upstage_last_kernel(const float *__restrict__ in, float *__restrict__ out,
                                                                const float *__restrict__ taps, int n_in, int s_rt, int indent)
{
    constexpr int TQ = 64;
    __shared__ float tile[TQ][PFEAT + 1];
    const int s = S > 0 ? S : s_rt;
    const long n_out = (long)n_in * s, nq = n_out - 2L * indent;
    for (long q0 = (long)blockIdx.x * TQ; q0 < nq; q0 += (long)gridDim.x * TQ) {
        for (int e = threadIdx.x; e < TQ * PFEAT; e += 256) {
            const int c = e / TQ, ql = e % TQ;
            const long q = q0 + ql + indent;
            float acc = 0.f;
            if (q0 + ql < nq) {
#pragma unroll
                for (int j = 0; j <= 2 * s; ++j) {
                    const long u = q + j - s;
                    float v = 0.f;
                    if (u >= 0 && u < n_out) v = in[(size_t)c * n_in + (int)(u / s)];
                    acc = fmaf(taps[j], v, acc);
                }
            }
            tile[ql][c] = acc;
        }
        __syncthreads();
        for (int e = threadIdx.x; e < TQ * PFEAT; e += 256) {
            const int ql = e / PFEAT, c = e % PFEAT;
            if (q0 + ql < nq) out[(size_t)(q0 + ql) * PFEAT + c] = tile[ql][c];
        }
        __syncthreads();
    }
}

}

using namespace wrnn;

static thread_local char g_pre_err[384] = "";
extern "C" const char *wrnn_pre_last_error(void) { return g_pre_err; }
#define PRE_FAIL(code, ...)                                  \
    do {                                                     \
        snprintf(g_pre_err, sizeof g_pre_err, __VA_ARGS__);  \
        return code;                                         \
    } while (0)
#define PRE_HIP(expr)                                                                                   \
    do {                                                                                                \
        hipError_t e_ = (expr);                                                                         \
        if (e_ != hipSuccess) PRE_FAIL(WRNN_ERR_HIP, "%s failed: %s", #expr, hipGetErrorString(e_));    \
    } while (0)

struct wrnn_pre {
    int device, blocks, scales[3], total_scale;
    int feat, C, R, pad;
    int gf;
    float *dev;
    const float *conv_in_w, *bn_in, *res_w, *res_bn, *conv_out_w, *conv_out_b, *taps[3];
};

static size_t generic_lds_bytes(int feat, int C, int pad, int gf) { return ((size_t)feat * (gf + 2 * pad) + 2 * (size_t)gf * C) * sizeof(float); }

extern "C" int wrnn_pre_create(const wrnn_pre_weights *w, int device, wrnn_pre **out)
{
    if (!w || !out) PRE_FAIL(WRNN_ERR_ARG, "NULL argument");
    if (w->feat_dims < 1 || w->feat_dims > 4096 || w->compute_dims < 1 || w->compute_dims > 4096 || w->res_out_dims < 1 || w->res_out_dims > 4096 ||
        w->pad < 0 || w->pad > 64 || w->res_blocks < 0 || w->res_blocks > 64)
        PRE_FAIL(WRNN_ERR_ARG, "bad UpsampleNetwork dims: feat_dims %d, compute_dims %d, res_out_dims %d, pad %d, res_blocks %d", w->feat_dims,
                 w->compute_dims, w->res_out_dims, w->pad, w->res_blocks);
    for (int i = 0; i < 3; ++i)
        if (w->upsample_factors[i] < 1 || w->upsample_factors[i] > 64) PRE_FAIL(WRNN_ERR_ARG, "bad upsample factor %d", w->upsample_factors[i]);
    if (!w->conv_in_w || !w->bn_in || (w->res_blocks && (!w->res_w || !w->res_bn)) || !w->conv_out_w || !w->conv_out_b || !w->up_w)
        PRE_FAIL(WRNN_ERR_ARG, "NULL weight pointer");
    const int FE = w->feat_dims, C = w->compute_dims, R = w->res_out_dims, PD = w->pad, KT = 2 * PD + 1;
    const bool shipped_dims = FE == PFEAT && C == PC && R == PC && PD == PPAD;
    int gf = 0;
    if (!shipped_dims) {
        for (gf = 16; gf >= 1 && generic_lds_bytes(FE, C, PD, gf) > 65536; gf >>= 1) {}
        if (gf < 1) PRE_FAIL(WRNN_ERR_ARG, "UpsampleNetwork too wide for the pre-loop kernel (feat_dims %d, compute_dims %d, pad %d)", FE, C, PD);
    }
    int n = 0;
    if (hipGetDeviceCount(&n) != hipSuccess || n <= 0 || device >= n) PRE_FAIL(WRNN_ERR_NO_DEVICE, "no HIP device %d (count %d)", device, n);
    DeviceGuard dg(device);
    PRE_HIP(dg.err);
    const int B = w->res_blocks;
    const double eps = 1e-5;
    std::vector<float> h;
    auto put = [&](const float *src, size_t cnt) { size_t o = (h.size() + 63) / 64 * 64; h.resize(o + cnt); if (src) memcpy(h.data() + o, src, cnt * 4); return o; };
    auto fold = [&](const float *bn, size_t o) {
        for (int c = 0; c < C; ++c) {
            const float s = bn[c] / sqrtf(bn[3 * C + c] + (float)eps);
            h[o + c] = s;
            h[o + C + c] = bn[C + c] - bn[2 * C + c] * s;
        }
    };
    const size_t o_cin = put(w->conv_in_w, (size_t)C * FE * KT);
    const size_t o_bnin = put(nullptr, 2 * (size_t)C);
    fold(w->bn_in, o_bnin);
    const size_t o_resw = put(w->res_w, (size_t)B * 2 * C * C);
    const size_t o_resbn = put(nullptr, (size_t)B * 2 * 2 * C);
    for (int i = 0; i < 2 * B; ++i) fold(w->res_bn + (size_t)i * 4 * C, o_resbn + (size_t)i * 2 * C);
    const size_t o_cow = put(w->conv_out_w, (size_t)R * C), o_cob = put(w->conv_out_b, R);
    size_t o_t[3], toff = 0;
    for (int i = 0; i < 3; ++i) { o_t[i] = put(w->up_w + toff, 2 * w->upsample_factors[i] + 1); toff += 2 * w->upsample_factors[i] + 1; }
    put(nullptr, 64);
    wrnn_pre *p = new wrnn_pre();
    p->device = device; p->blocks = B; p->total_scale = 1;
    p->feat = FE; p->C = C; p->R = R; p->pad = PD; p->gf = gf;
    for (int i = 0; i < 3; ++i) { p->scales[i] = w->upsample_factors[i]; p->total_scale *= w->upsample_factors[i]; }
    hipError_t e = hipMalloc((void **)&p->dev, h.size() * 4);
    if (e != hipSuccess) { delete p; PRE_FAIL(WRNN_ERR_HIP, "hipMalloc failed: %s", hipGetErrorString(e)); }
    e = hipMemcpy(p->dev, h.data(), h.size() * 4, hipMemcpyHostToDevice);
    if (e != hipSuccess) { (void)hipFree(p->dev); delete p; PRE_FAIL(WRNN_ERR_HIP, "hipMemcpy failed: %s", hipGetErrorString(e)); }
    p->conv_in_w = p->dev + o_cin; p->bn_in = p->dev + o_bnin; p->res_w = p->dev + o_resw; p->res_bn = p->dev + o_resbn;
    p->conv_out_w = p->dev + o_cow; p->conv_out_b = p->dev + o_cob;
    for (int i = 0; i < 3; ++i) p->taps[i] = p->dev + o_t[i];
    *out = p;
    return WRNN_OK;
}

extern "C" void wrnn_pre_destroy(wrnn_pre *p)
{
    if (!p) return;
    (void)hipFree(p->dev);
    delete p;
}

extern "C" int wrnn_pre_hop(const wrnn_pre *p) { return p ? p->total_scale : 0; }

extern "C" size_t wrnn_pre_workspace_bytes(const wrnn_pre *p, int32_t n_frames)
{
    if (!p || n_frames < 1) return 0;
    const size_t nf = (size_t)n_frames + 2 * p->pad;
    return (nf * p->scales[0] + nf * p->scales[0] * p->scales[1]) * p->feat * sizeof(float) + 512;
}

static int pre_run(const wrnn_pre *p, const float *mel, int32_t n_frames, float *mels_up, float *aux,
                   void *workspace, size_t workspace_bytes, void *stream_, bool rows_only)
{
    if (!p || !mel || !mels_up || !aux || !workspace) PRE_FAIL(WRNN_ERR_ARG, "NULL argument");
    if (n_frames < 1 || (double)n_frames * p->total_scale > 2.0e9) PRE_FAIL(WRNN_ERR_ARG, "bad n_frames %d", n_frames);
    if (workspace_bytes < wrnn_pre_workspace_bytes(p, n_frames)) PRE_FAIL(WRNN_ERR_WORKSPACE, "workspace too small");
    if (((uintptr_t)workspace & 255) != 0) PRE_FAIL(WRNN_ERR_ARG, "workspace must be 256-byte aligned");
    hipStream_t stream = (hipStream_t)stream_;
    DeviceGuard dg(p->device);
    PRE_HIP(dg.err);
    PreArgs a;
    a.mel = mel; a.conv_in_w = p->conv_in_w; a.bn_in = p->bn_in; a.res_w = p->res_w; a.res_bn = p->res_bn;
    a.conv_out_w = p->conv_out_w; a.conv_out_b = p->conv_out_b; a.aux = aux; a.N = n_frames; a.blocks = p->blocks;
    const int FE = p->feat, PD = p->pad;
    if (p->gf == 0) hipLaunchKernelGGL(wrnn_resnet_kernel, dim3((n_frames + PNF - 1) / PNF), dim3(256), 0, stream, a);
    else {
        GenPreArgs g;
        g.p = a; g.feat = FE; g.C = p->C; g.R = p->R; g.pad = PD; g.gf = p->gf;
        hipLaunchKernelGGL(wrnn_resnet_generic_kernel, dim3((n_frames + p->gf - 1) / p->gf), dim3(256), generic_lds_bytes(FE, p->C, PD, p->gf), stream, g);
    }
    const int nf = n_frames + 2 * PD;
    float *s1 = (float *)workspace;
    float *s2 = s1 + (size_t)nf * p->scales[0] * FE;
    auto grid = [](long total) { long b = (total + 255) / 256; return (unsigned)(b > 65535 ? 65535 : (b < 1 ? 1 : b)); };
    const bool feat80 = FE == PFEAT;
    const bool shipped = feat80 && PD == PPAD && p->scales[0] == 5 && p->scales[1] == 5 && p->scales[2] == 11;
    const unsigned g1 = grid((long)nf * p->scales[0] * FE), g2 = grid((long)nf * p->scales[0] * p->scales[1] * FE);
    const unsigned g3 = grid((long)n_frames * p->total_scale * 4);
    const int n2 = nf * p->scales[0], n3 = n2 * p->scales[1], indent = PD * p->total_scale;
    if (rows_only) {
        if (shipped) {
            hipLaunchKernelGGL((wrnn_upstage_kernel<true, false, 5>), dim3(g1), dim3(256), 0, stream, mel, s1, p->taps[0], nf, 5, PD, 0, PFEAT);
            hipLaunchKernelGGL((wrnn_upstage_kernel<false, true, 5>), dim3(g2), dim3(256), 0, stream, s1, mels_up, p->taps[1], n2, 5, 0, 0, PFEAT);
        } else {
            hipLaunchKernelGGL((wrnn_upstage_kernel<true, false, 0, 0>), dim3(g1), dim3(256), 0, stream, mel, s1, p->taps[0], nf, p->scales[0], PD, 0, FE);
            hipLaunchKernelGGL((wrnn_upstage_kernel<false, true, 0, 0>), dim3(g2), dim3(256), 0, stream, s1, mels_up, p->taps[1], n2, p->scales[1], 0, 0, FE);
        }
    } else if (shipped) {
        hipLaunchKernelGGL((wrnn_upstage_kernel<true, false, 5>), dim3(g1), dim3(256), 0, stream, mel, s1, p->taps[0], nf, 5, PD, 0, PFEAT);
        hipLaunchKernelGGL((wrnn_upstage_kernel<false, false, 5>), dim3(g2), dim3(256), 0, stream, s1, s2, p->taps[1], n2, 5, 0, 0, PFEAT);
        hipLaunchKernelGGL((wrnn_upstage_last_kernel<11>), dim3(g3), dim3(256), 0, stream, s2, mels_up, p->taps[2], n3, 11, indent);
    } else {
        hipLaunchKernelGGL((wrnn_upstage_kernel<true, false, 0, 0>), dim3(g1), dim3(256), 0, stream, mel, s1, p->taps[0], nf, p->scales[0], PD, 0, FE);
        hipLaunchKernelGGL((wrnn_upstage_kernel<false, false, 0, 0>), dim3(g2), dim3(256), 0, stream, s1, s2, p->taps[1], n2, p->scales[1], 0, 0, FE);
        if (feat80) hipLaunchKernelGGL((wrnn_upstage_last_kernel<0>), dim3(g3), dim3(256), 0, stream, s2, mels_up, p->taps[2], n3, p->scales[2], indent);
        else hipLaunchKernelGGL((wrnn_upstage_kernel<false, true, 0, 0>), dim3(grid((long)n_frames * p->total_scale * FE)), dim3(256), 0, stream, s2, mels_up, p->taps[2], n3, p->scales[2], 0, indent, FE);
    }
    PRE_HIP(hipGetLastError());
    return WRNN_OK;
}

extern "C" int wrnn_pre_upsample(const wrnn_pre *p, const float *mel, int32_t n_frames, float *mels_up, float *aux,
                                 void *workspace, size_t workspace_bytes, void *stream)
{
    return pre_run(p, mel, n_frames, mels_up, aux, workspace, workspace_bytes, stream, false);
}

extern "C" int wrnn_pre_upsample_rows(const wrnn_pre *p, const float *mel, int32_t n_frames, float *mel_rows, float *aux,
                                      void *workspace, size_t workspace_bytes, void *stream)
{
    return pre_run(p, mel, n_frames, mel_rows, aux, workspace, workspace_bytes, stream, true);
}
```

### wavernn_amd/pre.py

```python
import ctypes

import numpy as np
import torch

from . import _lib


def _f32(v):
    if isinstance(v, torch.Tensor):
        v = v.detach().to('cpu', torch.float32).numpy()
    return np.ascontiguousarray(v, dtype=np.float32)


class PreEngine:

    def __init__(self, state_dict, device=None):
        if not torch.cuda.is_available():
            raise _lib.WrnnError('wavernn_amd needs a HIP device; there is no CPU fallback')
        self.lib = _lib.lib()
        self.device = torch.device('cuda', torch.cuda.current_device()) if device is None else torch.device(device)
        sd = state_dict
        conv_in = _f32(sd['upsample.resnet.conv_in.weight'])
        C, feat, k = conv_in.shape
        blocks = 0
        while f'upsample.resnet.layers.{blocks}.conv1.weight' in sd:
            blocks += 1
        bn = lambda p: np.stack([_f32(sd[p + s]) for s in ('.weight', '.bias', '.running_mean', '.running_var')])
        res_w = np.stack([np.stack([_f32(sd[f'upsample.resnet.layers.{i}.conv{j}.weight'])[:, :, 0] for j in (1, 2)])
                          for i in range(blocks)]) if blocks else np.zeros((0, 2, C, C), np.float32)
        res_bn = np.stack([np.stack([bn(f'upsample.resnet.layers.{i}.batch_norm{j}') for j in (1, 2)])
                           for i in range(blocks)]) if blocks else np.zeros((0, 2, 4, C), np.float32)
        conv_out_w = _f32(sd['upsample.resnet.conv_out.weight'])[:, :, 0]
        ups = [_f32(sd[f'upsample.up_layers.{2 * i + 1}.weight']).reshape(-1) for i in range(3)]
        scales = [(u.shape[0] - 1) // 2 for u in ups]
        host = dict(conv_in_w=np.ascontiguousarray(conv_in.reshape(C, feat * k)), bn_in=np.ascontiguousarray(bn('upsample.resnet.batch_norm')),
                    res_w=np.ascontiguousarray(res_w), res_bn=np.ascontiguousarray(res_bn), conv_out_w=np.ascontiguousarray(conv_out_w),
                    conv_out_b=_f32(sd['upsample.resnet.conv_out.bias']), up_w=np.ascontiguousarray(np.concatenate(ups)))
        w = _lib.PreWeights()
        w.feat_dims, w.compute_dims, w.res_out_dims, w.res_blocks, w.pad = feat, C, conv_out_w.shape[0], blocks, (k - 1) // 2
        for i in range(3):
            w.upsample_factors[i] = scales[i]
        for name, arr in host.items():
            setattr(w, name, arr.ctypes.data)
        self.feat_dims, self.res_out_dims = int(feat), int(conv_out_w.shape[0])
        self.pad, self.scales, self.last_taps = int(w.pad), [int(s_) for s_ in scales], ups[2].copy()
        pre = ctypes.c_void_p()
        rc = self.lib.wrnn_pre_create(ctypes.byref(w), (self.device.index if self.device.index is not None else torch.cuda.current_device()), ctypes.byref(pre))
        if rc != 0:
            raise _lib.WrnnError(f'wrnn_pre_create failed (rc={rc}): {self.lib.wrnn_pre_last_error().decode()}')
        self._pre = pre
        self.hop = int(self.lib.wrnn_pre_hop(pre))
        self._ws = None

    def __del__(self):
        try:
            if getattr(self, '_pre', None):
                self.lib.wrnn_pre_destroy(self._pre)
                self._pre = None
        except Exception:
            pass

    def upsample_rows(self, mel, rows=None, aux=None):
        return self.upsample(mel, mels_up=rows, aux=aux, _rows=True)

    def rows_of(self, n_frames):
        return (int(n_frames) + 2 * self.pad) * self.scales[0] * self.scales[1]

    def upsample(self, mel, mels_up=None, aux=None, _rows=False):
        if mel.dim() == 3:
            mel = mel[0]
        mel = mel.to(self.device, torch.float32).contiguous()
        n = int(mel.shape[1])
        if mel.shape[0] != self.feat_dims:
            raise ValueError(f'Expected a mel shaped ({self.feat_dims}, n_hops), but got {tuple(mel.shape)}!')
        n_out = self.rows_of(n) if _rows else n * self.hop
        if mels_up is None:
            mels_up = torch.empty(n_out, self.feat_dims, dtype=torch.float32, device=self.device)
        if aux is None:
            aux = torch.empty(n, self.res_out_dims, dtype=torch.float32, device=self.device)
        assert mels_up.is_contiguous() and aux.is_contiguous() and mels_up.shape == (n_out, self.feat_dims)
        nbytes = int(self.lib.wrnn_pre_workspace_bytes(self._pre, n))
        stream = torch.cuda.current_stream(self.device).cuda_stream
        if self._ws is None:
            self._ws = {}
        ws = self._ws.get(stream)
        if ws is None or ws.numel() < nbytes:
            ws = self._ws[stream] = torch.empty(nbytes, dtype=torch.uint8, device=self.device)
        fn = self.lib.wrnn_pre_upsample_rows if _rows else self.lib.wrnn_pre_upsample
        rc = fn(self._pre, mel.data_ptr(), n, mels_up.data_ptr(), aux.data_ptr(), ws.data_ptr(), ws.numel(), stream)
        if rc != 0:
            raise _lib.WrnnError(f'wrnn_pre_upsample failed (rc={rc}): {self.lib.wrnn_pre_last_error().decode()}')
        return mels_up, aux

    def upsample_many(self, jobs, rows=False, streams=8):
        if streams <= 1 or len(jobs) <= 1:
            for mel, up, aux in jobs:
                self.upsample(mel, mels_up=up, aux=aux, _rows=rows)
            return
        cur = torch.cuda.current_stream(self.device)
        if getattr(self, '_side', None) is None or len(self._side) < streams:
            self._side = [torch.cuda.Stream(device=self.device) for _ in range(streams)]
        mels = [mel[0] if mel.dim() == 3 else mel for mel, _, _ in jobs]
        mels = [m.to(self.device, torch.float32).contiguous() for m in mels]
        fork = cur.record_event()
        used = self._side[:min(streams, len(jobs))]
        for s in used:
            s.wait_event(fork)
        for k, (m, (_, up, aux)) in enumerate(zip(mels, jobs)):
            with torch.cuda.stream(used[k % len(used)]):
                self.upsample(m, mels_up=up, aux=aux, _rows=rows)
        for s in used:
            cur.wait_stream(s)
```

Baseline: 10.75 million.

## Batch upsample jobs into single launches, fuse slab prep kernels, enlarge MoL tables

New measurement: 10.83 million, median of 6. No clear change (+0.7%).

```diff
diff --git a/include/wavernn_amd.h b/include/wavernn_amd.h
--- a/include/wavernn_amd.h
+++ b/include/wavernn_amd.h
@@ -154,6 +154,16 @@
                       void *workspace, size_t workspace_bytes, void *stream);
 int wrnn_pre_upsample_rows(const wrnn_pre *p, const float *mel, int32_t n_frames, float *mel_rows, float *aux,
                            void *workspace, size_t workspace_bytes, void *stream);
+typedef struct wrnn_pre_job {
+    const float *mel;
+    int32_t n_frames;
+    int64_t up_offset;
+    int64_t aux_offset;
+} wrnn_pre_job;
+int wrnn_pre_check_jobs(const wrnn_pre_weights *dims, const wrnn_pre_job *jobs, int32_t n_jobs, int32_t rows);
+size_t wrnn_pre_workspace_bytes_many(const wrnn_pre *p, const wrnn_pre_job *jobs, int32_t n_jobs, int32_t rows);
+int wrnn_pre_upsample_many(const wrnn_pre *p, const wrnn_pre_job *jobs, int32_t n_jobs, int32_t rows, float *mels_up, float *aux,
+                           void *workspace, size_t workspace_bytes, void *stream);
 const char *wrnn_pre_last_error(void);
 
 int wrnn_post_unfold(const float *segments, int32_t T, int32_t n_utt, const int32_t *first, const int32_t *folds,
diff --git a/wavernn_amd/_lib.py b/wavernn_amd/_lib.py
--- a/wavernn_amd/_lib.py
+++ b/wavernn_amd/_lib.py
@@ -17,7 +17,8 @@
            'wrnn_pack_weight_bytes', 'wrnn_pack_sparse_blocks', 'wrnn_pack_sparse_fc_blocks', 'wrnn_workspace_bytes', 'wrnn_workspace_bytes_segments', 'wrnn_generate',
            'wrnn_generate_segments', 'wrnn_plan_segments', 'wrnn_status', 'wrnn_timer_create', 'wrnn_timer_destroy', 'wrnn_timer_ms',
            'wrnn_timer_launches', 'wrnn_debug_read_exchange', 'wrnn_selftest', 'wrnn_selftest_metric', 'wrnn_pre_create',
-           'wrnn_pre_destroy', 'wrnn_pre_hop', 'wrnn_pre_workspace_bytes', 'wrnn_pre_upsample', 'wrnn_pre_upsample_rows', 'wrnn_pre_last_error',
+           'wrnn_pre_destroy', 'wrnn_pre_hop', 'wrnn_pre_workspace_bytes', 'wrnn_pre_upsample', 'wrnn_pre_upsample_rows', 'wrnn_pre_check_jobs', 'wrnn_pre_workspace_bytes_many',
+           'wrnn_pre_upsample_many', 'wrnn_pre_last_error',
            'wrnn_post_unfold', 'wrnn_post_last_error', 'wrnn_taco_workspace_bytes', 'wrnn_taco_decode', 'wrnn_taco_status',
            'wrnn_taco_last_error', 'wrnn_bigru']
 
@@ -32,6 +33,10 @@
     _fields_ = [(n, ctypes.c_int32) for n in ('feat_dims', 'compute_dims', 'res_out_dims', 'res_blocks', 'pad')] + \
                [('upsample_factors', ctypes.c_int32 * 3)] + \
                [(n, ctypes.c_void_p) for n in ('conv_in_w', 'bn_in', 'res_w', 'res_bn', 'conv_out_w', 'conv_out_b', 'up_w')]
+
+
+class PreJob(ctypes.Structure):
+    _fields_ = [('mel', ctypes.c_void_p), ('n_frames', ctypes.c_int32), ('up_offset', ctypes.c_int64), ('aux_offset', ctypes.c_int64)]
 
 
 TACO_WEIGHT_FIELDS = ('prenet_fc1_w', 'prenet_fc1_b', 'prenet_fc2_w', 'prenet_fc2_b', 'attn_rnn_w_ih', 'attn_rnn_w_hh', 'attn_rnn_b_ih',
@@ -157,6 +162,11 @@
     L.wrnn_pre_upsample.argtypes = [ctypes.c_void_p, ctypes.c_void_p, ctypes.c_int32, ctypes.c_void_p, ctypes.c_void_p,
                                     ctypes.c_void_p, ctypes.c_size_t, ctypes.c_void_p]
     L.wrnn_pre_upsample_rows.argtypes = L.wrnn_pre_upsample.argtypes
+    L.wrnn_pre_check_jobs.argtypes = [ctypes.POINTER(PreWeights), ctypes.POINTER(PreJob), ctypes.c_int32, ctypes.c_int32]
+    L.wrnn_pre_workspace_bytes_many.argtypes = [ctypes.c_void_p, ctypes.POINTER(PreJob), ctypes.c_int32, ctypes.c_int32]
+    L.wrnn_pre_workspace_bytes_many.restype = ctypes.c_size_t
+    L.wrnn_pre_upsample_many.argtypes = [ctypes.c_void_p, ctypes.POINTER(PreJob), ctypes.c_int32, ctypes.c_int32, ctypes.c_void_p, ctypes.c_void_p,
+                                         ctypes.c_void_p, ctypes.c_size_t, ctypes.c_void_p]
     L.wrnn_pre_last_error.restype = ctypes.c_char_p
     L.wrnn_post_unfold.argtypes = [ctypes.c_void_p, ctypes.c_int32, ctypes.c_int32, ctypes.c_void_p, ctypes.c_void_p, ctypes.c_void_p,
                                    ctypes.c_void_p, ctypes.c_int32, ctypes.c_void_p, ctypes.c_void_p, ctypes.c_int32,
diff --git a/wavernn_amd/csrc/wrnn_abi.hip b/wavernn_amd/csrc/wrnn_abi.hip
--- a/wavernn_amd/csrc/wrnn_abi.hip
+++ b/wavernn_amd/csrc/wrnn_abi.hip
@@ -16,6 +16,8 @@
 hipError_t launch_cond_frames_slab(const CondArgs &a, hipStream_t stream);
 hipError_t launch_cond_frag(const CondArgs &a, int n_cus, hipStream_t stream);
 hipError_t launch_noise_mol(const float *in, float *out, long n, int B, int n_cus, hipStream_t stream);
+hipError_t launch_slab_prep(const CondArgs &c, unsigned *xcc, void *ring, size_t ring_bytes, const float *nin, float *nout, long n_noise, int n_cus,
+                            hipStream_t stream);
 hipError_t launch_stream(const LoopArgs &args, int mode, hipStream_t stream);
 hipError_t launch_loop(const LoopArgs &args, int ncl, int mode, hipStream_t stream);
 int loop_max_depth(int mode);
@@ -414,7 +416,14 @@
 }
 
 enum Kind { K_STREAM, K_LOOP, K_SPARSE, K_DUO, K_GENERIC, K_CHAIN };
-constexpr int DUO_TAB_FPS = 8;
+constexpr int TAB_FPS_MIN = 8, TAB_FPS_MAX = 20;
+constexpr size_t SLAB_TAB_BYTES = 48u << 20, SLAB_NOISE_BYTES = 48u << 20;
+int plan_tab_fps(int B, int mode)
+{
+    if (mode != WRNN_MODE_MOL) return TAB_FPS_MIN;
+    const size_t fps = SLAB_TAB_BYTES / ((size_t)B * 5 * H * sizeof(float));
+    return fps < (size_t)TAB_FPS_MIN ? TAB_FPS_MIN : fps > (size_t)TAB_FPS_MAX ? TAB_FPS_MAX : (int)fps;
+}
 constexpr bool DUO_AUTO = true;
 constexpr int CHAIN_AUTO_GROUPS = 8;
 constexpr bool OCTO_AUTO = false;
@@ -495,13 +504,13 @@
         if (pl->ngr_max > ccl * g) { pl->rounds += 1; pl->per_round = (B + pl->rounds - 1) / pl->rounds; pl->ngr_max = (pl->per_round + SEG - 1) / SEG; }
         int slab = o->slab_steps;
         if (slab < 1) {
-            slab = p->mode == WRNN_MODE_MOL ? (int)((32u << 20) / ((size_t)pl->per_round * 11 * sizeof(float) * pl->rounds)) : 4096;
+            slab = p->mode == WRNN_MODE_MOL ? (int)(SLAB_NOISE_BYTES / ((size_t)pl->per_round * 11 * sizeof(float) * pl->rounds)) : 4096;
             if (slab < 16) slab = 16;
             if (slab > 4096) slab = 4096;
         }
         if (slab > T) slab = T;
         pl->slab = slab;
-        pl->tab_fps = DUO_TAB_FPS;
+        pl->tab_fps = plan_tab_fps(B, p->mode);
     }
     const int scl = sparse_clusters(p->n_cus);
     if (algo == WRNN_ALGO_SPARSE && (!p->sp_nbp || scl < 1)) {
@@ -518,13 +527,13 @@
         if (pl->ngr_max > scl) { pl->rounds += 1; pl->per_round = (B + pl->rounds - 1) / pl->rounds; pl->ngr_max = (pl->per_round + SEG - 1) / SEG; }
         int slab = o->slab_steps;
         if (slab < 1) {
-            slab = p->mode == WRNN_MODE_MOL ? (int)((32u << 20) / ((size_t)pl->per_round * 11 * sizeof(float) * pl->rounds)) : 4096;
+            slab = p->mode == WRNN_MODE_MOL ? (int)(SLAB_NOISE_BYTES / ((size_t)pl->per_round * 11 * sizeof(float) * pl->rounds)) : 4096;
             if (slab < 16) slab = 16;
             if (slab > 4096) slab = 4096;
         }
         if (slab > T) slab = T;
         pl->slab = slab;
-        pl->tab_fps = DUO_TAB_FPS;
+        pl->tab_fps = plan_tab_fps(B, p->mode);
     } else if (algo == WRNN_ALGO_AUTO || algo == WRNN_ALGO_LOOP || algo == WRNN_ALGO_DUO || algo == WRNN_ALGO_OCTO) {
         int ncl = loop_clusters(p->n_cus);
         if (algo == WRNN_ALGO_OCTO && (p->mode != WRNN_MODE_MOL || octo_clusters(p->n_cus) != MAXCL)) {
@@ -558,14 +567,14 @@
             if (pl->ngr_max > ncl * g) { pl->rounds += 1; pl->per_round = (B + pl->rounds - 1) / pl->rounds; pl->ngr_max = (pl->per_round + SEG - 1) / SEG; }
             int slab = o->slab_steps;
             if (slab < 1) {
-                if (pl->kind == K_DUO) slab = p->mode == WRNN_MODE_MOL ? (int)((32u << 20) / ((size_t)pl->per_round * 11 * sizeof(float) * pl->rounds)) : 4096;
+                if (pl->kind == K_DUO) slab = p->mode == WRNN_MODE_MOL ? (int)(SLAB_NOISE_BYTES / ((size_t)pl->per_round * 11 * sizeof(float) * pl->rounds)) : 4096;
                 else slab = (int)((96u << 20) / ((size_t)pl->ngr_max * SEG * H * sizeof(float)));
                 if (slab < 16) slab = 16;
                 if (slab > (pl->kind == K_DUO ? 4096 : 1024)) slab = pl->kind == K_DUO ? 4096 : 1024;
             }
             if (slab > T) slab = T;
             pl->slab = slab;
-            pl->tab_fps = DUO_TAB_FPS;
+            pl->tab_fps = plan_tab_fps(B, p->mode);
         } else if (algo == WRNN_ALGO_LOOP) {
             set_err("the loop kernel needs >= 64 CUs and (MOL or RAW with 512 classes); device has %d CUs, C=%d", p->n_cus, p->C);
             return WRNN_ERR_RESIDENCY;
@@ -823,17 +832,20 @@
         for (int s0 = pl.t0; s0 < pl.t1; s0 += pl.slab) {
             const int s1 = s0 + pl.slab < pl.t1 ? s0 + pl.slab : pl.t1;
             if (mol) {
-                HIPCHK(launch_noise_mol(noise + (size_t)(s0 - pl.t0) * 11 * B, (float *)(ws + l.npre), (long)(s1 - s0) * 11 * B, B, p->n_cus, stream));
                 a.noise_pre = (const float *)(ws + l.npre);
                 a.noise_t0 = s0;
             } else {
                 a.noise_t0 = pl.t0;
             }
+            const float *nz_in = mol ? noise + (size_t)(s0 - pl.t0) * 11 * B : nullptr;
+            const long nz_n = mol ? (long)(s1 - s0) * 11 * B : 0;
             if (duo) {
                 c.t0 = s0; c.B = B; c.FPS = pl.tab_fps;
-                HIPCHK(launch_cond_frames_slab(c, stream));
+                const size_t ring_bytes = (s0 == 0 || pl.rounds > 1 || (o->tuning & 4)) ? (chain ? chain_xbuf_bytes(pl.G) : sparse ? sparse_xbuf_bytes() : duo_xbuf_bytes(pl.G)) : 0;
+                HIPCHK(launch_slab_prep(c, (unsigned *)(ws + l.xcc), ws + l.xbuf, ring_bytes, nz_in, (float *)(ws + l.npre), nz_n, p->n_cus, stream));
                 a.tab_fps = pl.tab_fps; a.tab_t0 = s0;
-            }
+            } else if (mol) HIPCHK(launch_noise_mol(nz_in, (float *)(ws + l.npre), nz_n, B, p->n_cus, stream));
+            bool prepped = duo;
             for (int r = 0; r < pl.rounds; ++r) {
                 const int rb0 = (int)(((long)r * B) / pl.rounds), rb1 = (int)(((long)(r + 1) * B) / pl.rounds);
                 const int nr = rb1 - rb0;
@@ -842,8 +854,9 @@
                 c.t0 = s0; c.t1 = s1; c.rb0 = rb0; c.B = nr; c.NG = ngr;
                 if (!duo) HIPCHK(launch_cond_frag(c, p->n_cus, stream));
                 if (!duo) HIPCHK(hipMemsetAsync(ws + l.xbuf, 0xFF, XBUF_FLOATS * sizeof(float), stream));
-                else if (s0 == 0 || pl.rounds > 1 || (o->tuning & 4)) HIPCHK(hipMemsetAsync(ws + l.xbuf, 0xFF, chain ? chain_xbuf_bytes(pl.G) : sparse ? sparse_xbuf_bytes() : duo_xbuf_bytes(pl.G), stream));
-                if (duo) HIPCHK(hipMemsetAsync(ws + l.xcc, 0, XCC_WORDS * sizeof(unsigned), stream));
+                else if (!prepped && (s0 == 0 || pl.rounds > 1 || (o->tuning & 4))) HIPCHK(hipMemsetAsync(ws + l.xbuf, 0xFF, chain ? chain_xbuf_bytes(pl.G) : sparse ? sparse_xbuf_bytes() : duo_xbuf_bytes(pl.G), stream));
+                if (duo && !prepped) HIPCHK(hipMemsetAsync(ws + l.xcc, 0, XCC_WORDS * sizeof(unsigned), stream));
+                prepped = false;
                 a.state = (float *)(ws + l.state) + (size_t)r * (sparse ? sparse_state_floats() : chain ? chain_state_floats(pl.G) : loop_state_floats(pl.G));
                 a.t0 = s0; a.t1 = s1; a.cI_t0 = s0; a.rb0 = rb0; a.Btot = nr; a.NG = ngr; a.resume = s0 > 0 ? 1 : 0;
                 a.kind_tag = chain ? 4 : sparse ? 3 : (duo ? (octo ? 5 : 2) : 1);
diff --git a/wavernn_amd/csrc/wrnn_cond.hip b/wavernn_amd/csrc/wrnn_cond.hip
--- a/wavernn_amd/csrc/wrnn_cond.hip
+++ b/wavernn_amd/csrc/wrnn_cond.hip
@@ -200,10 +200,8 @@
     a.c4f[(size_t)f * H + r] = y4 + a.fc2_b[r];
 }
 
-__global__ __launch_bounds__(H) void wrnn_cond_frame_slab_kernel(const CondArgs a)
-{
-    __shared__ float ax[4 * AUX];
-    const int row = blockIdx.x, r = threadIdx.x;
+__device__ __forceinline__ void cond_frame_slab_row(const CondArgs &a, int row, int r, float *ax)
+{
     int f = a.NF;
     if (row < a.B * a.FPS) {
         const int b = row / a.FPS, j = row % a.FPS;
@@ -226,15 +224,63 @@
     a.c3f[(size_t)row * H + r] = y3 + a.fc1_b[r];
     a.c4f[(size_t)row * H + r] = y4 + a.fc2_b[r];
 }
-
+__global__ __launch_bounds__(H) void wrnn_cond_frame_slab_kernel(const CondArgs a)
+{
+    __shared__ float ax[4 * AUX];
+    cond_frame_slab_row(a, blockIdx.x, threadIdx.x, ax);
+}
+
+__device__ __forceinline__ float noise_mol_one(float u, long i, int B)
+{
+    const int col = (int)(i % (11L * B));
+    return (col < 10 * B) ? logf(-logf(u)) : (logf(u) - logf(1.0f - u));
+}
 __global__ __launch_bounds__(256) void wrnn_noise_mol_kernel(const float *__restrict__ in, float *__restrict__ out, long n, int B)
 {
     const long stride = (long)gridDim.x * blockDim.x;
-    for (long i = (long)blockIdx.x * blockDim.x + threadIdx.x; i < n; i += stride) {
-        const float u = in[i];
-        const int col = (int)(i % (11L * B));
-        out[i] = (col < 10 * B) ? logf(-logf(u)) : (logf(u) - logf(1.0f - u));
-    }
+    for (long i = (long)blockIdx.x * blockDim.x + threadIdx.x; i < n; i += stride) out[i] = noise_mol_one(in[i], i, B);
+}
+
+struct SlabPrepArgs {
+    CondArgs c;
+    unsigned *xcc;
+    uint4 *ring; long ring_n;
+    const float *nin; float *nout; long nn; int nB;
+    unsigned ring_blocks, noise_blocks;
+};
+static_assert(XCC_WORDS <= H, "one block zeroes the placement table");
+__global__ __launch_bounds__(H) void wrnn_slab_prep_kernel(const SlabPrepArgs s)
+{
+    __shared__ float ax[4 * AUX];
+    const unsigned rows = (unsigned)(s.c.B * s.c.FPS + 1);
+    unsigned blk = blockIdx.x;
+    if (blk < rows) { cond_frame_slab_row(s.c, (int)blk, threadIdx.x, ax); return; }
+    blk -= rows;
+    if (blk == 0) { if (threadIdx.x < XCC_WORDS) s.xcc[threadIdx.x] = 0u; return; }
+    blk -= 1;
+    if (blk < s.ring_blocks) {
+        const uint4 ff = make_uint4(0xFFFFFFFFu, 0xFFFFFFFFu, 0xFFFFFFFFu, 0xFFFFFFFFu);
+        for (long i = (long)blk * H + threadIdx.x; i < s.ring_n; i += (long)s.ring_blocks * H) s.ring[i] = ff;
+        return;
+    }
+    blk -= s.ring_blocks;
+    const long stride = (long)s.noise_blocks * H;
+    for (long i = (long)blk * H + threadIdx.x; i < s.nn; i += stride) s.nout[i] = noise_mol_one(s.nin[i], i, s.nB);
+}
+
+hipError_t launch_slab_prep(const CondArgs &c, unsigned *xcc, void *ring, size_t ring_bytes, const float *nin, float *nout, long n_noise, int n_cus,
+                            hipStream_t stream)
+{
+    if (ring_bytes % 16 != 0) return hipErrorInvalidValue;
+    SlabPrepArgs s;
+    s.c = c; s.xcc = xcc; s.ring = (uint4 *)ring; s.ring_n = (long)(ring_bytes / 16);
+    s.nin = nin; s.nout = nout; s.nn = n_noise; s.nB = c.B;
+    long rb = (s.ring_n + H - 1) / H, nb = (n_noise + H - 1) / H;
+    if (rb > n_cus) rb = n_cus;
+    if (nb > (long)n_cus * 4) nb = (long)n_cus * 4;
+    s.ring_blocks = (unsigned)rb; s.noise_blocks = (unsigned)nb;
+    hipLaunchKernelGGL(wrnn_slab_prep_kernel, dim3((unsigned)(c.B * c.FPS + 1) + 1u + s.ring_blocks + s.noise_blocks), dim3(H), 0, stream, s);
+    return hipGetLastError();
 }
 
 hipError_t launch_noise_mol(const float *in, float *out, long n, int B, int n_cus, hipStream_t stream)
diff --git a/wavernn_amd/csrc/wrnn_pre.hip b/wavernn_amd/csrc/wrnn_pre.hip
--- a/wavernn_amd/csrc/wrnn_pre.hip
+++ b/wavernn_amd/csrc/wrnn_pre.hip
@@ -1,6 +1,8 @@
 #include <math.h>
 #include <stdio.h>
 #include <string.h>
+#include <algorithm>
+#include <utility>
 #include <vector>
 
 #include "wrnn_device.h"
@@ -49,21 +51,17 @@
     return total;
 }
 
-__global__ __launch_bounds__(256) void wrnn_resnet_kernel(const PreArgs a)
-{
-    __shared__ __attribute__((aligned(16))) float XIN[PNF * PLDI];
-    __shared__ __attribute__((aligned(16))) float XA[PNF * PLDX];
-    __shared__ __attribute__((aligned(16))) float XB[PNF * PLDX];
+__device__ __forceinline__ void resnet_tile(const PreArgs &a, const float *__restrict__ mel, float *__restrict__ aux, const int N, const int j0,
+                                            float *XIN, float *XA, float *XB)
+{
     const int tid = threadIdx.x, lane = tid & 63, w = tid >> 6;
-    const int j0 = blockIdx.x * PNF;
-    const int N = a.N;
     for (int q = tid; q < PNF * PLDI; q += 256) {
         const int j = q / PLDI, k = q % PLDI;
         float v = 0.f;
         if (k < PKIN) {
             const int c = k / PK, t = k % PK;
             const int f = j0 + j + t - PPAD;
-            if (f >= 0 && f < N && j0 + j < N) v = a.mel[(size_t)c * N + f];
+            if (f >= 0 && f < N && j0 + j < N) v = mel[(size_t)c * N + f];
         }
         XIN[q] = v;
     }
@@ -117,8 +115,43 @@
         const f32x4 d = pre_tile(a.conv_out_w, PC, PC, row0, 1, XA, PLDX, lane);
         const float4 bo = *reinterpret_cast<const float4 *>(a.conv_out_b + row0 + rq);
         if (j0 + fi < N)
-            *reinterpret_cast<float4 *>(a.aux + (size_t)(j0 + fi) * PC + row0 + rq) = make_float4(d[0] + bo.x, d[1] + bo.y, d[2] + bo.z, d[3] + bo.w);
-    }
+            *reinterpret_cast<float4 *>(aux + (size_t)(j0 + fi) * PC + row0 + rq) = make_float4(d[0] + bo.x, d[1] + bo.y, d[2] + bo.z, d[3] + bo.w);
+    }
+}
+
+__global__ __launch_bounds__(256) void wrnn_resnet_kernel(const PreArgs a)
+{
+    __shared__ __attribute__((aligned(16))) float XIN[PNF * PLDI];
+    __shared__ __attribute__((aligned(16))) float XA[PNF * PLDX];
+    __shared__ __attribute__((aligned(16))) float XB[PNF * PLDX];
+    resnet_tile(a, a.mel, a.aux, a.N, blockIdx.x * PNF, XIN, XA, XB);
+}
+
+struct PreJobDev {
+    const float *mel;
+    float *up, *aux, *s1, *s2;
+    int N, b_res, b1, b2, b3;
+};
+enum { PJ_RES = 0, PJ_S1, PJ_S2, PJ_S3 };
+template <int WHICH>
+__device__ __forceinline__ int pre_job_of(const PreJobDev *__restrict__ jobs, int n_jobs, int blk)
+{
+    auto first = [&](int u) { return WHICH == PJ_RES ? jobs[u].b_res : WHICH == PJ_S1 ? jobs[u].b1 : WHICH == PJ_S2 ? jobs[u].b2 : jobs[u].b3; };
+    int lo = 0, hi = n_jobs - 1;
+    while (lo < hi) {
+        const int mid = (lo + hi + 1) >> 1;
+        if (first(mid) <= blk) lo = mid; else hi = mid - 1;
+    }
+    return lo;
+}
+
+__global__ __launch_bounds__(256) void wrnn_resnet_many_kernel(const PreArgs a, const PreJobDev *__restrict__ jobs, int n_jobs)
+{
+    __shared__ __attribute__((aligned(16))) float XIN[PNF * PLDI];
+    __shared__ __attribute__((aligned(16))) float XA[PNF * PLDX];
+    __shared__ __attribute__((aligned(16))) float XB[PNF * PLDX];
+    const int u = pre_job_of<PJ_RES>(jobs, n_jobs, blockIdx.x);
+    resnet_tile(a, jobs[u].mel, jobs[u].aux, jobs[u].N, (blockIdx.x - jobs[u].b_res) * PNF, XIN, XA, XB);
 }
 
 struct GenPreArgs {
@@ -173,6 +206,33 @@
     }
 }
 
+template <bool FIRST, bool LAST, int S, int F>
+__device__ __forceinline__ void upstage_elem(const float *__restrict__ in, float *__restrict__ out, const float *__restrict__ taps, int n_in, int s_rt,
+                                             int pad, int indent, int feat_rt, const long idx)
+{
+    const int s = S > 0 ? S : s_rt;
+    const int feat = F > 0 ? F : feat_rt;
+    const long n_out = (long)n_in * s;
+    const int ld_in = FIRST ? n_in - 2 * pad : n_in;
+    int c;
+    long q;
+    if (LAST) { c = (int)(idx % feat); q = idx / feat + indent; }
+    else { c = (int)(idx / n_out); q = idx % n_out; }
+    float acc = 0.f;
+#pragma unroll
+    for (int j = 0; j <= 2 * s; ++j) {
+        const long u = q + j - s;
+        float v = 0.f;
+        if (u >= 0 && u < n_out) {
+            int f = (int)(u / s);
+            if (FIRST) { f -= pad; v = (f >= 0 && f < ld_in) ? in[(size_t)c * ld_in + f] : 0.f; }
+            else v = in[(size_t)c * ld_in + f];
+        }
+        acc = fmaf(taps[j], v, acc);
+    }
+    if (LAST) out[(size_t)(q - indent) * feat + c] = acc;
+    else out[(size_t)c * n_out + q] = acc;
+}
 template <bool FIRST, bool LAST, int S, int F = PFEAT>
 __global__ __launch_bounds__(256) void wrnn_upstage_kernel(const float *__restrict__ in, float *__restrict__ out,
                                                            const float *__restrict__ taps, int n_in, int s_rt, int pad, int indent, int feat_rt = PFEAT)
@@ -181,62 +241,71 @@
     const int feat = F > 0 ? F : feat_rt;
     const long n_out = (long)n_in * s;
     const long total = LAST ? (n_out - 2L * indent) * feat : n_out * feat;
-    const int ld_in = FIRST ? n_in - 2 * pad : n_in;
-    for (long idx = (long)blockIdx.x * blockDim.x + threadIdx.x; idx < total; idx += (long)gridDim.x * blockDim.x) {
-        int c;
-        long q;
-        if (LAST) { c = (int)(idx % feat); q = idx / feat + indent; }
-        else { c = (int)(idx / n_out); q = idx % n_out; }
+    for (long idx = (long)blockIdx.x * blockDim.x + threadIdx.x; idx < total; idx += (long)gridDim.x * blockDim.x)
+        upstage_elem<FIRST, LAST, S, F>(in, out, taps, n_in, s_rt, pad, indent, feat_rt, idx);
+}
+template <int STAGE, bool ROWS, int S>
+__global__ __launch_bounds__(256) void wrnn_upstage_many_kernel(const PreJobDev *__restrict__ jobs, int n_jobs, const float *__restrict__ taps, int pad, int s0)
+{
+    const int u = pre_job_of<STAGE == 1 ? PJ_S1 : PJ_S2>(jobs, n_jobs, blockIdx.x);
+    const int nf = jobs[u].N + 2 * pad;
+    const int n_in = STAGE == 1 ? nf : nf * s0;
+    const long idx = (long)(blockIdx.x - (STAGE == 1 ? jobs[u].b1 : jobs[u].b2)) * 256 + threadIdx.x;
+    if (idx >= (long)n_in * S * PFEAT) return;
+    if (STAGE == 1) upstage_elem<true, false, S, PFEAT>(jobs[u].mel, jobs[u].s1, taps, n_in, S, pad, 0, PFEAT, idx);
+    else if (ROWS) upstage_elem<false, true, S, PFEAT>(jobs[u].s1, jobs[u].up, taps, n_in, S, 0, 0, PFEAT, idx);
+    else upstage_elem<false, false, S, PFEAT>(jobs[u].s1, jobs[u].s2, taps, n_in, S, 0, 0, PFEAT, idx);
+}
+
+constexpr int UPQ = 64;
+template <int S>
+__device__ __forceinline__ void upstage_last_tile(const float *__restrict__ in, float *__restrict__ out, const float *__restrict__ taps, int n_in, int s_rt,
+                                                  int indent, const long q0, float (*tile)[PFEAT + 1])
+{
+    constexpr int TQ = UPQ;
+    const int s = S > 0 ? S : s_rt;
+    const long n_out = (long)n_in * s, nq = n_out - 2L * indent;
+    for (int e = threadIdx.x; e < TQ * PFEAT; e += 256) {
+        const int c = e / TQ, ql = e % TQ;
+        const long q = q0 + ql + indent;
         float acc = 0.f;
-#pragma unroll
-        for (int j = 0; j <= 2 * s; ++j) {
-            const long u = q + j - s;
-            float v = 0.f;
-            if (u >= 0 && u < n_out) {
-                int f = (int)(u / s);
-                if (FIRST) { f -= pad; v = (f >= 0 && f < ld_in) ? in[(size_t)c * ld_in + f] : 0.f; }
-                else v = in[(size_t)c * ld_in + f];
+        if (q0 + ql < nq) {
+#pragma unroll
+            for (int j = 0; j <= 2 * s; ++j) {
+                const long u = q + j - s;
+                float v = 0.f;
+                if (u >= 0 && u < n_out) v = in[(size_t)c * n_in + (int)(u / s)];
+                acc = fmaf(taps[j], v, acc);
             }
-            acc = fmaf(taps[j], v, acc);
-        }
-        if (LAST) out[(size_t)(q - indent) * feat + c] = acc;
-        else out[(size_t)c * n_out + q] = acc;
-    }
+        }
+        tile[ql][c] = acc;
+    }
+    __syncthreads();
+    for (int e = threadIdx.x; e < TQ * PFEAT; e += 256) {
+        const int ql = e / PFEAT, c = e % PFEAT;
+        if (q0 + ql < nq) out[(size_t)(q0 + ql) * PFEAT + c] = tile[ql][c];
+    }
+    __syncthreads();
 }
 
 template <int S>
 __global__ __launch_bounds__(256) void wrnn_upstage_last_kernel(const float *__restrict__ in, float *__restrict__ out,
                                                                 const float *__restrict__ taps, int n_in, int s_rt, int indent)
 {
-    constexpr int TQ = 64;
-    __shared__ float tile[TQ][PFEAT + 1];
+    __shared__ float tile[UPQ][PFEAT + 1];
     const int s = S > 0 ? S : s_rt;
-    const long n_out = (long)n_in * s, nq = n_out - 2L * indent;
-    for (long q0 = (long)blockIdx.x * TQ; q0 < nq; q0 += (long)gridDim.x * TQ) {
-        for (int e = threadIdx.x; e < TQ * PFEAT; e += 256) {
-            const int c = e / TQ, ql = e % TQ;
-            const long q = q0 + ql + indent;
-            float acc = 0.f;
-            if (q0 + ql < nq) {
-#pragma unroll
-                for (int j = 0; j <= 2 * s; ++j) {
-                    const long u = q + j - s;
-                    float v = 0.f;
-                    if (u >= 0 && u < n_out) v = in[(size_t)c * n_in + (int)(u / s)];
-                    acc = fmaf(taps[j], v, acc);
-                }
-            }
-            tile[ql][c] = acc;
-        }
-        __syncthreads();
-        for (int e = threadIdx.x; e < TQ * PFEAT; e += 256) {
-            const int ql = e / PFEAT, c = e % PFEAT;
-            if (q0 + ql < nq) out[(size_t)(q0 + ql) * PFEAT + c] = tile[ql][c];
-        }
-        __syncthreads();
-    }
-}
-
+    const long nq = (long)n_in * s - 2L * indent;
+    for (long q0 = (long)blockIdx.x * UPQ; q0 < nq; q0 += (long)gridDim.x * UPQ) upstage_last_tile<S>(in, out, taps, n_in, s_rt, indent, q0, tile);
+}
+
+template <int S>
+__global__ __launch_bounds__(256) void wrnn_upstage_last_many_kernel(const PreJobDev *__restrict__ jobs, int n_jobs, const float *__restrict__ taps, int pad,
+                                                                     int s01, int indent)
+{
+    __shared__ float tile[UPQ][PFEAT + 1];
+    const int u = pre_job_of<PJ_S3>(jobs, n_jobs, blockIdx.x);
+    upstage_last_tile<S>(jobs[u].s2, jobs[u].up, taps, (jobs[u].N + 2 * pad) * s01, S, indent, (long)(blockIdx.x - jobs[u].b3) * UPQ, tile);
+}
 }
 
 using namespace wrnn;
@@ -400,3 +469,113 @@
 {
     return pre_run(p, mel, n_frames, mel_rows, aux, workspace, workspace_bytes, stream, true);
 }
+
+static int check_jobs(int feat, int R, int pad, const int *sc, const wrnn_pre_job *jobs, int32_t n_jobs, int32_t rows)
+{
+    if (!jobs) PRE_FAIL(WRNN_ERR_ARG, "NULL job table");
+    if (n_jobs < 1 || n_jobs > (1 << 20)) PRE_FAIL(WRNN_ERR_ARG, "bad n_jobs %d", n_jobs);
+    if (rows != 0 && rows != 1) PRE_FAIL(WRNN_ERR_ARG, "rows must be 0 or 1 (got %d)", rows);
+    const long hop = (long)sc[0] * sc[1] * sc[2];
+    std::vector<std::pair<int64_t, int64_t>> up(n_jobs), ax(n_jobs);
+    double blocks = 0;
+    for (int u = 0; u < n_jobs; ++u) {
+        const wrnn_pre_job &j = jobs[u];
+        if (!j.mel) PRE_FAIL(WRNN_ERR_ARG, "job %d: NULL mel", u);
+        if (j.n_frames < 1 || (double)j.n_frames * hop > 2.0e9) PRE_FAIL(WRNN_ERR_ARG, "job %d: bad n_frames %d", u, j.n_frames);
+        if (j.up_offset < 0 || j.aux_offset < 0) PRE_FAIL(WRNN_ERR_ARG, "job %d: negative output offset", u);
+        const int64_t n_up = rows ? (int64_t)(j.n_frames + 2 * pad) * sc[0] * sc[1] : (int64_t)j.n_frames * hop;
+        up[u] = {j.up_offset, j.up_offset + n_up * feat};
+        ax[u] = {j.aux_offset, j.aux_offset + (int64_t)j.n_frames * R};
+        blocks += ((double)(j.n_frames + 2 * pad) * sc[0] * sc[1] * feat + 255) / 256 + 1;
+    }
+    if (blocks > 2.0e9) PRE_FAIL(WRNN_ERR_ARG, "chunk too large for one launch (%.0f blocks); split it", blocks);
+    for (auto *v : {&up, &ax}) {
+        std::sort(v->begin(), v->end());
+        for (int u = 1; u < n_jobs; ++u)
+            if ((*v)[u].first < (*v)[u - 1].second) PRE_FAIL(WRNN_ERR_ARG, "overlapping %s outputs in the job table", v == &up ? "mels_up" : "aux");
+    }
+    return WRNN_OK;
+}
+
+extern "C" int wrnn_pre_check_jobs(const wrnn_pre_weights *dims, const wrnn_pre_job *jobs, int32_t n_jobs, int32_t rows)
+{
+    if (!dims) PRE_FAIL(WRNN_ERR_ARG, "NULL argument");
+    if (dims->feat_dims < 1 || dims->res_out_dims < 1 || dims->pad < 0 || dims->upsample_factors[0] < 1 || dims->upsample_factors[1] < 1 || dims->upsample_factors[2] < 1)
+        PRE_FAIL(WRNN_ERR_ARG, "bad UpsampleNetwork dims");
+    return check_jobs(dims->feat_dims, dims->res_out_dims, dims->pad, dims->upsample_factors, jobs, n_jobs, rows);
+}
+
+static bool pre_batched(const wrnn_pre *p)
+{
+    return p->gf == 0 && p->feat == PFEAT && p->pad == PPAD && p->scales[0] == 5 && p->scales[1] == 5 && p->scales[2] == 11;
+}
+static size_t many_table_bytes(int n_jobs) { return ((size_t)(n_jobs + 1) * sizeof(PreJobDev) + 255) / 256 * 256; }
+static size_t many_job_floats(const wrnn_pre *p, int n_frames, bool rows, size_t *s2_off)
+{
+    const size_t nf = (size_t)n_frames + 2 * p->pad;
+    const size_t f1 = (nf * p->scales[0] * p->feat + 63) / 64 * 64;
+    *s2_off = f1;
+    return f1 + (rows ? 0 : (nf * p->scales[0] * p->scales[1] * p->feat + 63) / 64 * 64);
+}
+
+extern "C" size_t wrnn_pre_workspace_bytes_many(const wrnn_pre *p, const wrnn_pre_job *jobs, int32_t n_jobs, int32_t rows)
+{
+    if (!p || !jobs || n_jobs < 1 || !pre_batched(p)) return 0;
+    size_t fl = 0, o;
+    for (int u = 0; u < n_jobs; ++u) {
+        if (jobs[u].n_frames < 1) return 0;
+        fl += many_job_floats(p, jobs[u].n_frames, rows != 0, &o);
+    }
+    return many_table_bytes(n_jobs) + fl * sizeof(float);
+}
+
+extern "C" int wrnn_pre_upsample_many(const wrnn_pre *p, const wrnn_pre_job *jobs, int32_t n_jobs, int32_t rows, float *mels_up, float *aux,
+                                      void *workspace, size_t workspace_bytes, void *stream_)
+{
+    if (!p || !mels_up || !aux || !workspace) PRE_FAIL(WRNN_ERR_ARG, "NULL argument");
+    int rc = check_jobs(p->feat, p->R, p->pad, p->scales, jobs, n_jobs, rows);
+    if (rc != WRNN_OK) return rc;
+    if (!pre_batched(p)) PRE_FAIL(WRNN_ERR_ARG, "this UpsampleNetwork runs the dimension-generic kernels, which take one utterance per call (wrnn_pre_upsample)");
+    if (workspace_bytes < wrnn_pre_workspace_bytes_many(p, jobs, n_jobs, rows)) PRE_FAIL(WRNN_ERR_WORKSPACE, "workspace too small");
+    if (((uintptr_t)workspace & 255) != 0) PRE_FAIL(WRNN_ERR_ARG, "workspace must be 256-byte aligned");
+    hipStream_t stream = (hipStream_t)stream_;
+    DeviceGuard dg(p->device);
+    PRE_HIP(dg.err);
+    const int PD = p->pad, s0 = p->scales[0], s1 = p->scales[1];
+    std::vector<PreJobDev> tab(n_jobs + 1);
+    float *base = (float *)((char *)workspace + many_table_bytes(n_jobs));
+    long b_res = 0, b1 = 0, b2 = 0, b3 = 0;
+    size_t fl = 0;
+    for (int u = 0; u <= n_jobs; ++u) {
+        PreJobDev &d = tab[u];
+        memset(&d, 0, sizeof d);
+        d.b_res = (int)b_res; d.b1 = (int)b1; d.b2 = (int)b2; d.b3 = (int)b3;
+        if (u == n_jobs) break;
+        const int N = jobs[u].n_frames;
+        const long nf = N + 2 * PD;
+        size_t s2_off;
+        const size_t mine = many_job_floats(p, N, rows != 0, &s2_off);
+        d.mel = jobs[u].mel; d.up = mels_up + jobs[u].up_offset; d.aux = aux + jobs[u].aux_offset; d.N = N;
+        d.s1 = base + fl; d.s2 = rows ? nullptr : base + fl + s2_off;
+        fl += mine;
+        b_res += (N + PNF - 1) / PNF;
+        b1 += (nf * s0 * PFEAT + 255) / 256;
+        b2 += (nf * s0 * s1 * PFEAT + 255) / 256;
+        b3 += ((long)N * p->total_scale + UPQ - 1) / UPQ;
+    }
+    PRE_HIP(hipMemcpyAsync(workspace, tab.data(), tab.size() * sizeof(PreJobDev), hipMemcpyHostToDevice, stream));
+    const PreJobDev *dj = (const PreJobDev *)workspace;
+    PreArgs a;
+    memset(&a, 0, sizeof a);
+    a.conv_in_w = p->conv_in_w; a.bn_in = p->bn_in; a.res_w = p->res_w; a.res_bn = p->res_bn;
+    a.conv_out_w = p->conv_out_w; a.conv_out_b = p->conv_out_b; a.blocks = p->blocks;
+    hipLaunchKernelGGL(wrnn_resnet_many_kernel, dim3((unsigned)b_res), dim3(256), 0, stream, a, dj, n_jobs);
+    hipLaunchKernelGGL((wrnn_upstage_many_kernel<1, false, 5>), dim3((unsigned)b1), dim3(256), 0, stream, dj, n_jobs, p->taps[0], PD, s0);
+    if (rows) hipLaunchKernelGGL((wrnn_upstage_many_kernel<2, true, 5>), dim3((unsigned)b2), dim3(256), 0, stream, dj, n_jobs, p->taps[1], PD, s0);
+    else {
+        hipLaunchKernelGGL((wrnn_upstage_many_kernel<2, false, 5>), dim3((unsigned)b2), dim3(256), 0, stream, dj, n_jobs, p->taps[1], PD, s0);
+        hipLaunchKernelGGL((wrnn_upstage_last_many_kernel<11>), dim3((unsigned)b3), dim3(256), 0, stream, dj, n_jobs, p->taps[2], PD, s0 * s1, PD * p->total_scale);
+    }
+    PRE_HIP(hipGetLastError());
+    return WRNN_OK;
+}
diff --git a/wavernn_amd/pre.py b/wavernn_amd/pre.py
--- a/wavernn_amd/pre.py
+++ b/wavernn_amd/pre.py
@@ -93,15 +93,39 @@
         return mels_up, aux
 
     def upsample_many(self, jobs, rows=False, streams=8):
+        if not jobs:
+            return
+        mels = [mel[0] if mel.dim() == 3 else mel for mel, _, _ in jobs]
+        mels = [m.to(self.device, torch.float32).contiguous() for m in mels]
+        tab = (_lib.PreJob * len(jobs))()
+        up0, aux0 = min(up.data_ptr() for _, up, _ in jobs), min(aux.data_ptr() for _, _, aux in jobs)
+        for k, (m, (_, up, aux)) in enumerate(zip(mels, jobs)):
+            n = int(m.shape[1])
+            if m.shape[0] != self.feat_dims:
+                raise ValueError(f'Expected a mel shaped ({self.feat_dims}, n_hops), but got {tuple(m.shape)}!')
+            assert up.is_contiguous() and aux.is_contiguous() and up.shape == (self.rows_of(n) if rows else n * self.hop, self.feat_dims)
+            assert aux.shape == (n, self.res_out_dims) and up.dtype == aux.dtype == torch.float32
+            tab[k].mel, tab[k].n_frames = m.data_ptr(), n
+            tab[k].up_offset, tab[k].aux_offset = (up.data_ptr() - up0) // 4, (aux.data_ptr() - aux0) // 4
+        nbytes = int(self.lib.wrnn_pre_workspace_bytes_many(self._pre, tab, len(jobs), int(bool(rows))))
+        if nbytes:
+            stream = torch.cuda.current_stream(self.device).cuda_stream
+            if self._ws is None:
+                self._ws = {}
+            ws = self._ws.get('many')
+            if ws is None or ws.numel() < nbytes:
+                ws = self._ws['many'] = torch.empty(nbytes, dtype=torch.uint8, device=self.device)
+            rc = self.lib.wrnn_pre_upsample_many(self._pre, tab, len(jobs), int(bool(rows)), up0, aux0, ws.data_ptr(), ws.numel(), stream)
+            if rc != 0:
+                raise _lib.WrnnError(f'wrnn_pre_upsample_many failed (rc={rc}): {self.lib.wrnn_pre_last_error().decode()}')
+            return
         if streams <= 1 or len(jobs) <= 1:
-            for mel, up, aux in jobs:
-                self.upsample(mel, mels_up=up, aux=aux, _rows=rows)
+            for m, (_, up, aux) in zip(mels, jobs):
+                self.upsample(m, mels_up=up, aux=aux, _rows=rows)
             return
         cur = torch.cuda.current_stream(self.device)
         if getattr(self, '_side', None) is None or len(self._side) < streams:
             self._side = [torch.cuda.Stream(device=self.device) for _ in range(streams)]
-        mels = [mel[0] if mel.dim() == 3 else mel for mel, _, _ in jobs]
-        mels = [m.to(self.device, torch.float32).contiguous() for m in mels]
         fork = cur.record_event()
         used = self._side[:min(streams, len(jobs))]
         for s in used:
```
